# Graph-Machine-Learning-Group/sgp

Hardware: AMD Instinct MI355X
Metric: encoded node-steps/sec (higher is better)
Workload: dtype f32 (hop products: operands as fp16 hi + lo pairs, three 16-bit MFMA terms per product, fp32 accumulation -- agrees with fp32 to ~1e-7 of the operand scale; reservoir: recurrent products: state (|h| <= 1, x 2^14) and W_hh (per-row power-of-two scale) as two fp16 pieces (22 bits), hi*hi + hi*lo + lo*

## Files before the change

### include/sgp_amd.h

```cpp
#ifndef SGP_AMD_H
#define SGP_AMD_H

#include <stdint.h>

#ifdef __cplusplus
extern "C" {
#endif

#define SGP_ABI_VERSION 4

#define SGP_EINVAL   (-1)
#define SGP_EUNSUP   (-2)
#define SGP_ENOMEM   (-3)

#define SGP_ACT_TANH      0
#define SGP_ACT_RELU      1
#define SGP_ACT_SELF_NORM 2
#define SGP_ACT_IDENTITY  3
#define SGP_ACT_TANH_REL  4

typedef void* sgp_stream_t;

int sgp_abi_version(void);
const char* sgp_last_error(void);
const char* sgp_build_arch(void);

int64_t sgp_tune_value(const char* key, int64_t dflt);

int sgp_spmm_csr_f32(const int32_t* rowptr, const int32_t* col, const float* val,
                     const float* X, int64_t x_row_stride, int64_t x_batch_stride,
                     const float* X_halo, int64_t xh_row_stride, int64_t xh_batch_stride,
                     int32_t n_own,
                     float* Y, int64_t y_row_stride, int64_t y_batch_stride,
                     int32_t n_rows, int32_t n_cols, int32_t batch, int32_t feat,
                     const int32_t* pred, int32_t run_if, sgp_stream_t stream);

int sgp_spmm_tiled_f32(const int32_t* tile_row_ptr, const int32_t* uptr, const int32_t* ucol,
                       const int32_t* erow, const uint16_t* ecol, const float* eval,
                       int32_t tile_rows, int32_t n_tiles,
                       int32_t max_union, int32_t max_row_edges,
                       const float* X, int64_t x_row_stride, int64_t x_batch_stride,
                       const float* X_halo, int64_t xh_row_stride, int64_t xh_batch_stride,
                       int32_t n_own,
                       float* Y, int64_t y_row_stride, int64_t y_batch_stride,
                       int32_t n_rows, int32_t n_cols, int32_t batch, int32_t feat,
                       const int32_t* pred, int32_t run_if, sgp_stream_t stream);
int sgp_spmm_res_f32(const int32_t* uptr, const int32_t* ucol, const int32_t* usplit,
                     const int32_t* gptr, const int32_t* gsup, const int32_t* gidx, const float* gw,
                     const int32_t* rowmap,
                     int32_t n_tiles, int32_t max_union, int32_t max_tile_quads,
                     const float* X, int64_t x_row_stride, int64_t x_batch_stride,
                     const float* X_halo, int64_t xh_row_stride, int64_t xh_batch_stride,
                     int32_t n_own,
                     float* Y, int64_t y_row_stride, int64_t y_batch_stride,
                     int32_t n_rows, int32_t n_cols, int32_t batch, int32_t feat,
                     const int32_t* pred, int32_t run_if, sgp_stream_t stream);
int32_t sgp_spmm_res_max_union(void);
int32_t sgp_spmm_res_max_quads(void);
int sgp_spmm_res_tune(int32_t cfg);

int sgp_spmm_mix_f32(const int32_t* uptr, const int32_t* ucol, const int32_t* usplit,
                     const int32_t* gptr, const int32_t* gsup, const int32_t* gidx, const float* gw,
                     const int32_t* rowmap,
                     const int32_t* dptr, const int32_t* didx, const float* dw,
                     int32_t n_tiles, int32_t max_union, int32_t max_dense,
                     const float* X, int64_t x_row_stride, int64_t x_batch_stride,
                     const float* X_halo, int64_t xh_row_stride, int64_t xh_batch_stride,
                     int32_t n_own,
                     float* Y, int64_t y_row_stride, int64_t y_batch_stride,
                     int32_t n_rows, int32_t n_cols, int32_t batch, int32_t feat,
                     const int32_t* pred, int32_t run_if, sgp_stream_t stream);
int32_t sgp_spmm_mix_max_union(void);
int32_t sgp_spmm_mix_max_dense(int32_t halo);

int sgp_abs_max_f32(const float* X, int64_t x_row_stride, int64_t x_batch_stride,
                    int32_t n_rows, int32_t batch, int32_t feat, float* out, sgp_stream_t stream);


int sgp_col_stats_f32(const float* X, int64_t x_row_stride, int64_t x_batch_stride,
                      int32_t n_rows, int32_t batch, int32_t feat, int32_t t_stride, int32_t r_stride, int32_t accumulate,
                      float* stats, sgp_stream_t stream);

int sgp_split_prepare_f32(const float* stats, double n_samples, double s_eff, int32_t full,
                          const float* bound_in, float bound_scalar, float norm_inf, int32_t feat,
                          float* x_tab, float* bound_out, int32_t* flag, sgp_stream_t stream);

int sgp_spmm_split_f32(const int32_t* hdr, const int32_t* rowid, const int32_t* ucol, const void* afr,
                       const int32_t* adr, const float* rinv, int32_t n_tiles,
                       const float* X, int64_t x_row_stride, int64_t x_batch_stride,
                       const float* X_halo, int64_t xh_row_stride, int64_t xh_batch_stride, int32_t n_own,
                       float* Y, int64_t y_row_stride, int64_t y_batch_stride,
                       int32_t n_rows, int32_t n_cols, int32_t batch, int32_t feat,
                       const float* x_tab, int32_t accumulate, int32_t t_chunk, const int32_t* pred, int32_t run_if, sgp_stream_t stream);
int32_t sgp_spmm_split_chunks(void);
int32_t sgp_spmm_split_max_union(void);
int32_t sgp_spmm_split_waves(void);
int32_t sgp_spmm_split_rows_per_wave(void);
int32_t sgp_spmm_split_max_feat(void);

int sgp_spmm_split_banded_f32(const int32_t* hdr, const int32_t* rowid, const int32_t* ucol, const void* afr,
                              const int32_t* adr, const float* rinv, int32_t n_tiles,
                              const float* X, int64_t x_row_stride, int64_t x_batch_stride,
                              const float* X_halo, int64_t xh_row_stride, int64_t xh_batch_stride, int32_t n_own,
                              float* Y, int64_t y_row_stride, int64_t y_batch_stride,
                              int32_t n_rows, int32_t n_cols, int32_t batch, int32_t feat,
                              const float* x_tab, int32_t accumulate, int32_t t_chunk,
                              int32_t walk, const int32_t* band_first, int32_t n_bands,
                              const int32_t* pred, int32_t run_if, sgp_stream_t stream);

int sgp_spmm_split_wide_f32(const int32_t* hdr, const int32_t* rowid, const int32_t* ucol, const void* afr,
                            const int32_t* adr, const float* rinv, int32_t n_tiles,
                            const float* X, int64_t x_row_stride, int64_t x_batch_stride,
                            const float* X_halo, int64_t xh_row_stride, int64_t xh_batch_stride, int32_t n_own,
                            float* Y, int64_t y_row_stride, int64_t y_batch_stride,
                            int32_t n_rows, int32_t n_cols, int32_t batch, int32_t feat,
                            const float* x_tab, int32_t accumulate, int32_t t_chunk, const int32_t* pred, int32_t run_if, sgp_stream_t stream);
int sgp_spmm_split_wide_banded_f32(const int32_t* hdr, const int32_t* rowid, const int32_t* ucol, const void* afr,
                                   const int32_t* adr, const float* rinv, int32_t n_tiles,
                                   const float* X, int64_t x_row_stride, int64_t x_batch_stride,
                                   const float* X_halo, int64_t xh_row_stride, int64_t xh_batch_stride, int32_t n_own,
                                   float* Y, int64_t y_row_stride, int64_t y_batch_stride,
                                   int32_t n_rows, int32_t n_cols, int32_t batch, int32_t feat,
                                   const float* x_tab, int32_t accumulate, int32_t t_chunk,
                                   int32_t walk, const int32_t* band_first, int32_t n_bands,
                                   const int32_t* pred, int32_t run_if, sgp_stream_t stream);
int32_t sgp_spmm_split_wide_chunks(void);
int32_t sgp_spmm_split_wide_max_union(void);
int32_t sgp_spmm_split_wide_waves(void);
int32_t sgp_spmm_split_wide_rows_per_wave(void);
int32_t sgp_spmm_split_wide_max_feat(void);

int sgp_split_plan_order(const int64_t* rowptr, const int64_t* col, int64_t nnz, int64_t n_rows, int64_t n_cols,
                         int32_t waves, int32_t chunks, int32_t max_union, int32_t rows_per_wave, int64_t* order);
int64_t sgp_split_plan_deal(const int64_t* rowptr, const int64_t* col, int64_t nnz, int64_t n_rows, int64_t n_cols,
                            const int64_t* order, int64_t n_order,
                            int32_t waves, int32_t chunks, int32_t max_union, int32_t rows_per_wave,
                            int64_t* wave_of_row, int64_t* slot_of_row, int64_t* tile_of_wave, int64_t* rows_of_wave);
int sgp_split_plan_fill(const int64_t* rowptr, const int64_t* col, const float* val, int64_t nnz, int64_t n_rows, int64_t n_cols,
                        const int64_t* wave_of_row, const int64_t* slot_of_row, const int64_t* tile_of_wave,
                        const int64_t* rows_of_wave, int64_t n_waves, int64_t n_tiles,
                        int32_t waves, int32_t chunks, int32_t max_union,
                        int32_t* hdr, int32_t* rowid, int32_t* ucol, void* afr, int32_t* adr, float* rinv,
                        double* stats, int32_t threads);
int64_t sgp_split_plan_bands(const int32_t* ucol, int64_t n_tiles, int32_t max_union, int64_t n_cols,
                             int64_t col_budget, int32_t* band_first);

int sgp_spmm_colblock_f32(const int32_t* plan, const int32_t* segptr, const int32_t* wg_row0,
                          int32_t n_wg, int32_t n_blocks,
                          const float* X, int64_t x_row_stride, int64_t x_batch_stride,
                          const float* X_halo, int64_t xh_row_stride, int64_t xh_batch_stride, int32_t n_own,
                          float* Y, int64_t y_row_stride, int64_t y_batch_stride,
                          int32_t n_rows, int32_t n_cols, int32_t batch, int32_t feat,
                          const int32_t* pred, int32_t run_if, sgp_stream_t stream);
int32_t sgp_spmm_colblock_rows_cap(void);
int32_t sgp_spmm_colblock_round_pad(void);

int32_t sgp_spmm_tiled_max_union(int32_t feat);
int32_t sgp_spmm_tiled_max_tile_rows(void);
int32_t sgp_spmm_tiled_max_row_edges(void);

int sgp_spmm_tiled_form(int32_t tile_rows, int32_t max_row_edges, int32_t* rows_per_group, int32_t* batches);
int32_t sgp_spmm_csr_form(int32_t feat, int32_t aligned, int32_t predicated);

int64_t sgp_reservoir_workspace_bytes(int32_t F, int32_t R);
int sgp_reservoir_f32(const float* x, int64_t x_row_stride, int64_t x_step_stride,
                      const float* w_ih, const float* w_hh, const float* b,
                      double alpha, int32_t act,
                      float* out, int64_t out_row_stride, int64_t out_step_stride,
                      float* h_state, void* workspace,
                      int32_t T, int32_t N, int32_t F, int32_t R,
                      sgp_stream_t stream);

int sgp_reservoir_pieces_f32(const float* x, int64_t x_row_stride, int64_t x_step_stride,
                             const float* w_ih, const float* w_hh, const float* b,
                             double alpha, int32_t act,
                             float* out, int64_t out_row_stride, int64_t out_step_stride,
                             float* h_state, void* workspace,
                             int32_t t_piece, int32_t t_last, int32_t n_pieces,
                             int64_t x_piece_stride, int64_t out_piece_stride, int32_t no_store,
                             int32_t N, int32_t F, int32_t R,
                             const int32_t* pred, int32_t run_if, sgp_stream_t stream);

int sgp_reservoir_describe(int32_t F, int32_t R, int32_t N, int32_t T, int32_t act, double alpha, int32_t has_state,
                           int32_t n_pieces, int32_t no_store, int32_t has_pred,
                           int64_t x_row_stride, int64_t x_step_stride, int32_t x_align,
                           int64_t out_row_stride, int64_t out_step_stride, int32_t out_align,
                           char* text, int64_t capacity);

int64_t sgp_reservoir_fused_workspace_bytes(int32_t F, int32_t R, int32_t L);
int32_t sgp_reservoir_fused_supported(int32_t F, int32_t R, int32_t L);
int sgp_reservoir_fused_f32(const float* x, int64_t x_row_stride, int64_t x_step_stride,
                            const float* const* w_ih, const float* const* w_hh, const float* const* b,
                            const double* alpha, int32_t act,
                            float* out, int64_t out_row_stride, int64_t out_step_stride,
                            float* h_state, void* workspace,
                            int32_t T, int32_t N, int32_t F, int32_t R, int32_t L,
                            sgp_stream_t stream);
int sgp_reservoir_fused_sums_f32(const float* x, int64_t x_row_stride, int64_t x_step_stride,
                                 const float* const* w_ih, const float* const* w_hh, const float* const* b,
                                 const double* alpha, int32_t act,
                                 float* out, int64_t out_row_stride, int64_t out_step_stride,
                                 float* h_state, void* workspace, float* tile_sums,
                                 int32_t T, int32_t N, int32_t F, int32_t R, int32_t L,
                                 sgp_stream_t stream);

int32_t sgp_reservoir_window_supported(int32_t F, int32_t R, int32_t L);
int64_t sgp_reservoir_window_workspace_bytes(int32_t F, int32_t R, int32_t L, int32_t S, int64_t M);
int sgp_reservoir_window_f32(const float* x, int64_t x_batch_stride, int64_t x_step_stride, int64_t x_node_stride, int32_t Fx,
                             const float* u, int64_t u_batch_stride, int64_t u_step_stride, int64_t u_node_stride, int32_t Fu,
                             const int32_t* step_start,
                             const float* const* w_ih, const float* const* w_hh, const float* const* b,
                             const double* alpha, int32_t act,
                             const float* h0, float* out, int64_t out_row_stride,
                             void* workspace, int32_t packed,
                             int32_t B, int32_t N, int32_t S, int32_t R, int32_t L, sgp_stream_t stream);

int64_t sgp_gesn_workspace_bytes(int32_t N, int32_t R, int32_t L);
int sgp_gesn_tune(int32_t persistent);
int sgp_gesn_f32(const int32_t* rowptr, const int32_t* col, const float* val,
                 const float* x, int64_t x_row_stride, int64_t x_step_stride,
                 const float* const* w_ih, const float* const* w_hh, const float* const* b,
                 const double* alpha, int32_t act,
                 float* out, int64_t out_row_stride, int64_t out_step_stride,
                 float* h_state, void* workspace,
                 int32_t T, int32_t N, int32_t F, int32_t R, int32_t L, sgp_stream_t stream);
int sgp_gemm_nt_f32(const float* A, int64_t lda, const float* W, int64_t ldw, const float* bias,
                    float* C, int64_t ldc, int32_t M, int32_t N, int32_t K, sgp_stream_t stream);
int sgp_gesn_update_f32(const int32_t* rowptr, const int32_t* col, const float* val,
                        const float* z, const float* p, const float* h_in,
                        double alpha, int32_t act,
                        float* h_out, float* out_row, int64_t out_stride,
                        int32_t n_nodes, int32_t R, sgp_stream_t stream);

int sgp_node_mean_bcast_f32(const float* X, int64_t x_row_stride, int64_t x_batch_stride,
                            float* Y, int64_t y_row_stride, int64_t y_batch_stride,
                            float* partial,
                            int32_t n_rows, int32_t batch, int32_t feat,
                            sgp_stream_t stream);
int sgp_bcast_rows_f32(const float* src, float scale,
                       float* Y, int64_t y_row_stride, int64_t y_batch_stride,
                       int32_t n_rows, int32_t batch, int32_t feat,
                       sgp_stream_t stream);

int sgp_copy_rows_f32(const float* X, int64_t x_row_stride, int64_t x_batch_stride,
                      float* Y, int64_t y_row_stride, int64_t y_batch_stride,
                      int32_t n_rows, int32_t batch, int32_t feat,
                      sgp_stream_t stream);
int sgp_gather_rows_f32(const float* X, int64_t x_row_stride, int64_t x_batch_stride,
                        const int32_t* step, const int32_t* node, int32_t n_index,
                        float* out, int64_t out_row_stride, int64_t out_batch_stride,
                        int32_t batch, int32_t feat, sgp_stream_t stream);

int64_t sgp_grouped_linear_packed_floats(int32_t groups, int32_t ic, int32_t oc);
int sgp_grouped_linear_pack_f32(const float* w, float* packed, int32_t groups, int32_t ic, int32_t oc,
                                sgp_stream_t stream);
int sgp_grouped_linear_f32(const float* X, int64_t x_row_stride, int64_t x_batch_stride,
                           const int32_t* step, const int32_t* node,
                           const float* w_packed, const float* bias, int32_t act,
                           float* out, int64_t out_row_stride,
                           int32_t n_rows, int32_t groups, int32_t ic, int32_t oc,
                           sgp_stream_t stream);
int sgp_grouped_linear_fwd_f32(const float* X, int64_t x_row_stride, int64_t x_batch_stride,
                               const int32_t* step, const int32_t* node,
                               const float* w_packed, const float* bias, int32_t act,
                               float* out, int64_t out_row_stride, float* pre,
                               double dropout_p, uint64_t seed,
                               int32_t n_rows, int32_t groups, int32_t ic, int32_t oc,
                               sgp_stream_t stream);
int sgp_grouped_linear_dact_f32(const float* dy, int64_t dy_row_stride, const float* pre, int32_t act,
                                double dropout_p, uint64_t seed,
                                float* dz, int64_t n_rows, int32_t width, sgp_stream_t stream);
int sgp_grouped_linear_transpose_f32(const float* w, float* wt, int32_t groups, int32_t ic, int32_t oc,
                                     sgp_stream_t stream);
int sgp_grouped_linear_wgrad_f32(const float* X, int64_t x_row_stride, int64_t x_batch_stride,
                                 const int32_t* step, const int32_t* node,
                                 const float* dz, float* dw,
                                 int32_t n_rows, int32_t groups, int32_t ic, int32_t oc,
                                 sgp_stream_t stream);
int sgp_grouped_linear_form(int32_t ic, int32_t oc, int64_t x_row_stride, int64_t x_batch_stride, int32_t x_aligned16,
                            int32_t* jtc, int32_t* xvec);
int sgp_grouped_linear_wgrad_form(int32_t n_rows, int32_t groups, int32_t ic, int32_t oc,
                                  int32_t* rows_per_slice, int32_t* slices);

int64_t sgp_ridge_workspace_bytes(int32_t which, int64_t n_rows, int32_t n_cols, int32_t n_out);
int sgp_ridge_form(int32_t which, int64_t n_rows, int32_t n_cols, int32_t n_out, int64_t* out);

int sgp_ridge_colmeans_f32(const int64_t* segs, int32_t n_segs, const int32_t* steps, int64_t n_steps,
                           int64_t n_nodes, double* means, void* work, int64_t work_bytes, sgp_stream_t stream);

int sgp_ridge_gram_f32(const int64_t* segs, int32_t n_segs, const int32_t* steps, int64_t n_steps, int64_t n_nodes,
                       const float* shift, int32_t ones, double* gram, int64_t ldg, void* work, int64_t work_bytes,
                       sgp_stream_t stream);

int sgp_ridge_predict_score_f32(const int64_t* segs, int32_t n_segs, const int32_t* steps, int64_t n_steps,
                                int64_t n_nodes, const float* W, const double* b, int32_t horizon, int32_t channels,
                                const float* scale, const float* bias, int64_t sc_node_stride,
                                const float* y, int64_t y_ss, int64_t y_ns,
                                const uint8_t* mask, int64_t m_ss, int64_t m_ns, int64_t m_cs,
                                float* yhat, double* sums, void* work, int64_t work_bytes, sgp_stream_t stream);


int64_t sgp_dense_packed_floats(int32_t n_out, int32_t k);
int sgp_dense_pack_f32(const float* w, int64_t w_row_stride, int32_t transpose, int32_t n_out, int32_t k,
                       float* packed, sgp_stream_t stream);

int sgp_dense_f32(const float* X, int64_t x_row_stride, const int32_t* gather, int64_t row_mod,
                  const float* w_packed, const float* bias, int32_t n_rows, int32_t k, int32_t n_out,
                  int32_t act, int32_t n_act, int32_t dmode, const float* dpre, int64_t dpre_row_stride,
                  float* pre, int64_t pre_row_stride, double dropout_p, uint64_t seed, int64_t drop_width,
                  const float* add, int64_t add_row_stride,
                  float* out, const int64_t* out_map, sgp_stream_t stream);
int sgp_dense_form(int32_t n_rows, int32_t n_out, int32_t k, int64_t x_row_stride, int32_t x_aligned16,
                   int32_t* rows_per_wg, int32_t* xvec);

int64_t sgp_dense_wgrad_workspace_floats(int64_t n_rows, int32_t n_out, int32_t k, int32_t with_bias);
int sgp_dense_wgrad_f32(const float* dZ, int64_t dz_row_stride, const float* X, int64_t x_row_stride,
                        const int32_t* gather, int64_t row_mod, int32_t n_rows, int32_t n_out, int32_t k,
                        float* dw, int64_t dw_row_stride, float* db, float* work, int64_t work_floats,
                        sgp_stream_t stream);

int sgp_row_segsum_f32(const float* g, int64_t g_row_stride, int64_t n_rows, int32_t width,
                       const int32_t* perm, const int32_t* keys, int32_t n_seg, float* out, sgp_stream_t stream);


int sgp_multi_sqnorm_f32(const int64_t* table, int64_t n_chunks, const float* const* grads, double* partial,
                         float* norm_f32, double* norm_f64, sgp_stream_t stream);

int sgp_adam_step_f32(const int64_t* table, int64_t n_chunks, float* const* params, const float* const* grads,
                      float* const* exp_avg, float* const* exp_avg_sq, const float* norm, double max_norm,
                      double lr, double beta1, double beta2, double eps, double weight_decay, int64_t step,
                      int32_t decoupled, sgp_stream_t stream);

int64_t sgp_masked_metrics_workspace_doubles(int64_t batch, int32_t horizon, int64_t nodes, int32_t channels);
int sgp_masked_metrics_f32(const float* y_hat, const float* y, const uint8_t* mask, int64_t batch, int32_t horizon,
                           int64_t nodes, int32_t channels, const float* scale, const float* bias,
                           int64_t sc_node_stride, int32_t mask_nans, int32_t mask_inf, double* work,
                           int64_t work_doubles, double* state, sgp_stream_t stream);

int64_t sgp_masked_loss_workspace_doubles(int64_t batch, int32_t horizon, int64_t row, int32_t at);
int sgp_masked_loss_f32(const float* y_hat, const float* y, const uint8_t* mask, int64_t batch, int32_t horizon,
                        int64_t row, int32_t kind, int32_t at, int32_t mask_nans, double* work, int64_t work_doubles,
                        float* loss, double* count, sgp_stream_t stream);
int sgp_masked_loss_bwd_f32(const float* y_hat, const float* y, const uint8_t* mask, int64_t batch, int32_t horizon,
                            int64_t row, int32_t kind, int32_t at, int32_t mask_nans, const float* grad_out,
                            const double* count, float* grad, sgp_stream_t stream);


int32_t sgp_gated_gn_supported(int32_t H, int32_t act);
int32_t sgp_gated_gn_chunk_edges(void);
int64_t sgp_gated_gn_workspace_bytes(int32_t backward, int64_t b, int64_t n_edges, int64_t n_chunks, int32_t n_parts,
                                     int32_t H);

int sgp_gated_gn_edge_f32(const float* PQ, int64_t pq_row_stride, int32_t b, int32_t n, int32_t H, int32_t act,
                          const int32_t* chunks, int32_t n_chunks, const int32_t* src, int64_t n_edges,
                          const int32_t* fix, int32_t n_fix, int32_t n_parts,
                          const float* w2_packed, const float* b2, const float* wg, const float* bg,
                          float* agg, int64_t agg_row_stride, void* work, int64_t work_bytes, sgp_stream_t stream);

int sgp_gated_gn_edge_bwd_f32(const float* PQ, int64_t pq_row_stride, const float* dAgg, int64_t dagg_row_stride,
                              int32_t b, int32_t n, int32_t H, int32_t act,
                              const int32_t* chunks, int32_t n_chunks, const int32_t* src, int64_t n_edges,
                              const int32_t* fix, int32_t n_fix, int32_t n_parts,
                              const int32_t* src_ptr, const int32_t* src_pos,
                              const float* w2_packed, const float* w2t_packed, const float* b2, const float* wg,
                              const float* bg, float* dPQ, int64_t dpq_row_stride, float* dW2, float* db2, float* dwg,
                              float* dbg, void* work, int64_t work_bytes, sgp_stream_t stream);

int32_t sgp_rnn_window_supported(int32_t cell, int32_t H);
int64_t sgp_rnn_window_packed_floats(int32_t cell, int32_t H);
int64_t sgp_rnn_window_workspace_bytes(int32_t cell, int32_t H, int32_t S, int64_t M);
int sgp_rnn_window_pack_f32(const float* w_hh, int32_t cell, int32_t H, float* packed, sgp_stream_t stream);

int sgp_rnn_window_fwd_f32(int32_t cell, int32_t H, int32_t S, int64_t M, float* gates, const float* packed,
                           const float* b_hn, float* h_seq, float* c_seq, float* h_drop, double dropout_p, uint64_t seed,
                           float* h_last, int32_t save, sgp_stream_t stream);

int sgp_rnn_window_bwd_f32(int32_t cell, int32_t H, int32_t S, int64_t M, float* gates, const float* packed,
                           const float* h_seq, const float* c_seq, const float* dy, int32_t dy_full,
                           sgp_stream_t stream);

int32_t sgp_dcrnn_supported(int32_t H, int32_t k);

int sgp_diffuse_f32(const int32_t* rowptr0, const int32_t* col0, const float* val0, int64_t xcol0, int64_t ycol0,
                    const int32_t* rowptr1, const int32_t* col1, const float* val1, int64_t xcol1, int64_t ycol1,
                    const float* X, int64_t x_row_stride, int64_t x_batch_stride,
                    float* Y, int64_t y_row_stride, int64_t y_batch_stride,
                    int32_t n, int32_t batch, int32_t feat, int32_t accumulate, sgp_stream_t stream);

int sgp_dcrnn_gates_f32(const float* Dh, int64_t d_row_stride, const float* w_ru_packed,
                        const float* G, int64_t g_row_stride, float* ruc, int64_t ruc_row_stride,
                        float* Drh, int64_t drh_row_stride, int64_t R, int32_t H, int32_t k, sgp_stream_t stream);

int sgp_dcrnn_update_f32(const float* Drh, int64_t d_row_stride, const float* w_c_packed,
                         const float* G, int64_t g_row_stride, float* ruc, int64_t ruc_row_stride,
                         const float* h_prev, int64_t h_row_stride, float* h_seq_t, float* dh_next,
                         int64_t dh_next_row_stride, float* h_last, int64_t R, int32_t H, int32_t k,
                         sgp_stream_t stream);

int sgp_dcrnn_bwd_f32(int32_t phase, float* dh, const float* ruc, int64_t ruc_row_stride,
                      const float* h_prev, int64_t h_row_stride, const float* dDrh, int64_t ddrh_row_stride,
                      float* dz, int64_t dz_row_stride, int64_t R, int32_t H, sgp_stream_t stream);

int32_t sgp_gwnet_supported(int32_t H, int32_t Kt);

int sgp_gwnet_tconv_f32(const float* X, int64_t x_row_stride, int64_t x_rows, int64_t tap_rows,
                        const float* w_packed, const float* bias, float* Y, int64_t y_row_stride,
                        float* act, int64_t act_row_stride, int64_t n_rows, int32_t H, int32_t Kt,
                        sgp_stream_t stream);

int sgp_gwnet_tconv_bwd_f32(const float* dY, int64_t dy_row_stride, float* act, int64_t act_row_stride,
                            int64_t n_rows, int32_t H, sgp_stream_t stream);

int sgp_adj_apply_f32(const float* A, int64_t a_row_stride, int32_t transpose,
                      const float* X, int64_t xcol, int64_t x_row_stride, int64_t x_batch_stride,
                      float* Y, int64_t ycol, int64_t y_row_stride, int64_t y_batch_stride,
                      int32_t n, int32_t batch, int32_t feat, int32_t accumulate, sgp_stream_t stream);

int64_t sgp_adj_grad_workspace_floats(int32_t n, int32_t batch);
int sgp_adj_grad_f32(const float* dY, int64_t dycol, int64_t dy_row_stride, int64_t dy_batch_stride,
                     const float* X, int64_t xcol, int64_t x_row_stride, int64_t x_batch_stride,
                     float* dA, int64_t da_row_stride, int32_t n, int32_t batch, int32_t feat, int32_t accumulate,
                     float* work, int64_t work_floats, sgp_stream_t stream);

int sgp_row_softmax_f32(const float* L, int64_t l_row_stride, float* A, int64_t a_row_stride, int32_t n_rows, int32_t n,
                        sgp_stream_t stream);
int sgp_row_softmax_bwd_f32(const float* A, int64_t a_row_stride, const float* dA, int64_t da_row_stride,
                            const float* L, int64_t l_row_stride, float* dL, int64_t dl_row_stride,
                            int32_t n_rows, int32_t n, sgp_stream_t stream);

int64_t sgp_gwnet_norm_workspace_doubles(int64_t R, int32_t H);
int sgp_gwnet_norm_f32(int32_t kind, int32_t training, const float* Y, int64_t y_row_stride,
                       const float* res, int64_t res_row_stride, double dropout_p, uint64_t seed,
                       const float* weight, const float* bias, float* running_mean, float* running_var,
                       double momentum, double eps, float* z_save, float* stats,
                       float* out, int64_t out_row_stride, int64_t R, int32_t H,
                       double* work, int64_t work_doubles, sgp_stream_t stream);

int sgp_gwnet_norm_bwd_f32(int32_t kind, int32_t training, const float* dOut, int64_t dout_row_stride,
                           const float* z, const float* stats, const float* weight, double dropout_p, uint64_t seed,
                           double eps, float* dY, int64_t dy_row_stride, float* dRes, int64_t dres_row_stride,
                           float* dweight, float* dbias, int64_t R, int32_t H,
                           double* work, int64_t work_doubles, sgp_stream_t stream);

int sgp_subgraph_mark(const int32_t* ids, int64_t n_ids, uint64_t* mask, int64_t n_nodes, int32_t* err,
                      sgp_stream_t stream);
int sgp_subgraph_expand(const int32_t* src, const int32_t* dst, int64_t n_edges, const uint64_t* mask_in,
                        uint64_t* mask_out, int64_t n_nodes, sgp_stream_t stream);
int sgp_subgraph_edge_flags(const int32_t* src, const int32_t* dst, int64_t n_edges, const uint64_t* mask,
                            int64_t n_nodes, uint64_t* flags, uint8_t* edge_mask, sgp_stream_t stream);

int64_t sgp_compact_tiles(int64_t n);
int sgp_compact_pack_u8(const uint8_t* flags, int64_t n, uint64_t* bits, sgp_stream_t stream);
int sgp_compact_count(const uint64_t* bits, int64_t n, int32_t* tile_offsets, int32_t* total, sgp_stream_t stream);
int sgp_compact_scatter(const uint64_t* bits, int64_t n, const int32_t* tile_offsets, int64_t n_set, int32_t* idx32,
                        int64_t* idx64, int32_t* rank, sgp_stream_t stream);
int sgp_subgraph_edges(const uint64_t* flags, int64_t n_edges, const int32_t* tile_offsets, int64_t n_set,
                       const int32_t* src, const int32_t* dst, const float* weight, const int32_t* relabel,
                       int64_t n_nodes, int64_t* out_src, int64_t* out_dst, float* out_weight, sgp_stream_t stream);
int sgp_subgraph_take_edges(const int32_t* src, const int32_t* dst, const float* weight, int64_t n_edges,
                            const int32_t* pos, int64_t n_pos, const int64_t* keep, int64_t n_keep,
                            const int32_t* relabel, int64_t n_nodes, int64_t* out_src, int64_t* out_dst,
                            float* out_weight, int32_t* err, sgp_stream_t stream);

int32_t sgp_conn_max_knn(void);
int sgp_conn_geo_knn_f64(const double* unit, int64_t n, int32_t k, int32_t include_self, int32_t binary,
                         double threshold, double chord_zero, double scale, int32_t* out_col, double* out_val,
                         sgp_stream_t stream);
int sgp_conn_geo_rows_f64(const double* unit, int64_t n, int32_t include_self, int32_t binary, double threshold,
                          double chord_lo, double chord_hi, double scale, int32_t* row_count, const int64_t* rowptr,
                          int32_t* out_col, double* out_val, sgp_stream_t stream);
int sgp_conn_dense_knn(const void* sim, int32_t is_f64, int64_t row_stride, int64_t col_stride, int64_t n, int32_t k,
                       int32_t include_self, int32_t binary, double threshold, int32_t* out_col, double* out_val,
                       sgp_stream_t stream);
int sgp_conn_dense_rows(const void* sim, int32_t is_f64, int64_t row_stride, int64_t col_stride, int64_t n,
                        int32_t include_self, int32_t binary, double threshold, int32_t* row_count,
                        const int64_t* rowptr, int32_t* out_col, double* out_val, sgp_stream_t stream);
int sgp_correntropy_f32(const float* x, int64_t x_row_stride, int32_t n, int32_t period, int32_t n_chunks, double gamma,
                        float* norms, float* out, int64_t out_row_stride, sgp_stream_t stream);

int64_t sgp_scaler_workspace_bytes(int64_t m, int64_t g, int32_t regime, int64_t rows_per_wg);
int sgp_scaler_moments_f32(const float* x, const uint8_t* mask, int64_t mask_div, int64_t m, int64_t g, int32_t want_var,
                           int32_t regime, int64_t rows_per_wg, int32_t tile_cols, double* stats, void* ws,
                           int64_t ws_bytes, sgp_stream_t stream);
int sgp_scaler_select_f32(const float* x, const uint8_t* mask, int64_t mask_div, int64_t m, int64_t g, const double* stats,
                          double q_lo, double q_mid, double q_hi, int32_t regime, int64_t rows_per_wg, int32_t tile_cols,
                          float* ostat, void* ws, int64_t ws_bytes, sgp_stream_t stream);
int sgp_scaler_finish_f32(int32_t kind, const double* stats, const float* ostat, int64_t g, int32_t has_mask, double p0,
                          double p1, double adjust, float* bias, float* scale, sgp_stream_t stream);
int sgp_scaler_apply_f32(const float* x, float* out, const float* bias, const float* scale, int64_t n, int64_t n_params,
                         int32_t inverse, sgp_stream_t stream);

int32_t sgp_edge_sort_tile(void);
int32_t sgp_edge_sort_passes(int64_t n_nodes);
int64_t sgp_edge_sort_workspace_bytes(int64_t n_items);
int sgp_edge_sort(const void* keys, int32_t keys64, int64_t n_keys, const int32_t* payload_in, int64_t n_items,
                  int64_t n_nodes, int32_t* order, int32_t* ptr, int32_t* err, void* ws, int64_t ws_bytes,
                  sgp_stream_t stream);
int sgp_edge_segment_sum_f32(const int32_t* ptr, const int32_t* order, const float* weight, int64_t n_nodes,
                             int64_t n_items, float* deg, sgp_stream_t stream);
int sgp_edge_gather_f32(const int32_t* order, int64_t n_items, const void* other, int32_t other64, const float* weight,
                        const void* idx_a, const float* deg_a, const void* idx_b, const float* deg_b, int32_t idx64,
                        int64_t n_nodes, int32_t* col, float* val_a, float* val_b, sgp_stream_t stream);
int sgp_edge_chunk_tables(const int32_t* ptr, int64_t n_nodes, int32_t chunk, int32_t* scan, int32_t* counts,
                          int32_t* chunks, int64_t max_chunks, int32_t* fix, int64_t max_fix, sgp_stream_t stream);

#define SGP_SHIFT_GCN_NORM    1
#define SGP_SHIFT_SET_DIAG    2
#define SGP_SHIFT_REMOVE_DIAG 4
#define SGP_SHIFT_UNDIRECTED  8
#define SGP_SHIFT_TRANSPOSE   16
int64_t sgp_shift_operator_workspace_bytes(int64_t n_items, int64_t n_nodes);
int sgp_shift_operator_f32(const void* src, const void* dst, int32_t idx64, const float* weight, int64_t n_edges,
                           int64_t n_nodes, int32_t flags, int32_t* rowptr, int32_t* col, float* val, int64_t capacity,
                           int32_t* nnz, int32_t* err, void* ws, int64_t ws_bytes, sgp_stream_t stream);

#define SGP_SPGEMM_COUNT 1
#define SGP_SPGEMM_EMIT  2
#define SGP_SPGEMM_ERR_CAPACITY 1
#define SGP_SPGEMM_ERR_INDEX    2
int64_t sgp_spgemm_workspace_bytes(int64_t n_rows);
int sgp_spgemm_form(int64_t n_rows, int64_t n_cols, int64_t* out);
int sgp_spgemm_f32(const int32_t* a_rowptr, const int32_t* a_col, const float* a_val, int64_t a_capacity, int64_t n_rows,
                   int64_t n_mid, const int32_t* b_rowptr, const int32_t* b_col, const float* b_val, int64_t b_capacity,
                   int64_t n_cols, int32_t phase, int32_t* rowptr, int32_t* col, float* val, int64_t capacity,
                   int32_t* nnz, int32_t* err, void* ws, int64_t ws_bytes, sgp_stream_t stream);
int sgp_csr_take_rows_f32(const int32_t* a_rowptr, const int32_t* a_col, const float* a_val, int64_t a_capacity,
                          int64_t n_rows, const void* index, int32_t idx64, int64_t n_index, int32_t phase,
                          int32_t* rowptr, int32_t* col, float* val, int64_t capacity, int32_t* nnz, int32_t* err, void* ws,
                          int64_t ws_bytes, sgp_stream_t stream);

int sgp_event_create(void** ev);
int sgp_event_destroy(void* ev);
int sgp_event_record(void* ev, sgp_stream_t stream);
int sgp_event_elapsed_ms(void* start, void* stop, float* ms);

#ifdef __cplusplus
}
#endif
#endif
```

### sgp_amd/csrc/plan_split.hip

```cpp
#include "common.h"
#include <math.h>
#include <string.h>
#include <algorithm>
#include <atomic>
#include <new>
#include <system_error>
#include <thread>
#include <vector>

namespace {

constexpr int SET_SLOTS[4][8] = {{0, 1, 2, 3, 8, 9, 10, 11}, {4, 5, 6, 7, 12, 13, 14, 15},
                                 {16, 17, 18, 19, 24, 25, 26, 27}, {20, 21, 22, 23, 28, 29, 30, 31}};

inline uint16_t half_bits(_Float16 h) { uint16_t b; memcpy(&b, &h, 2); return b; }

inline void split_fp16(float v, uint16_t& hi, uint16_t& lo) {
    uint32_t bits;
    memcpy(&bits, &v, 4);
    bits &= 0xFFFFE000u;
    float hi32;
    memcpy(&hi32, &bits, 4);
    if (fabsf(v) < 6.103515625e-05f) hi32 = (float)(_Float16)v;
    const _Float16 h = (_Float16)hi32;
    const _Float16 l = (_Float16)(v - (float)h);
    hi = half_bits(h);
    lo = half_bits(l);
}

inline int row_exponent(float rmax) {
    if (!(rmax > 0.0f)) return 0;
    const float q = 16384.0f / rmax;
    int e;
    if (isinf(q)) e = 126;
    else { int ex; (void)frexpf(q, &ex); e = ex - 1; }
    return std::min(126, std::max(-126, e));
}

struct FillArgs {
    const int64_t* rowptr; const int64_t* col; const float* val;
    int64_t n_rows, n_cols;
    const int64_t* wave_of_row; const int64_t* slot_of_row; const int64_t* tile_of_wave; const int64_t* rows_of_wave;
    int64_t n_waves, n_tiles;
    int waves, chunks, max_union;
    int32_t* hdr; int32_t* rowid; int32_t* ucol; uint16_t* afr; int32_t* adr; float* rinv;
};

struct Scratch {
    std::vector<int32_t> stage_of_col, kpos_of_col;
    std::vector<int64_t> cols;
    std::vector<float> dense;
    explicit Scratch(const FillArgs& a) : stage_of_col(a.n_cols, -1), kpos_of_col(a.n_cols, -1), dense((size_t)a.chunks * 512) {}
};

int64_t fill_tile(const FillArgs& a, int64_t t, const int64_t* first_wave, const int64_t* row_list, const int64_t* row_first,
                  Scratch& s, int64_t& union_out) {
    const int W = a.waves, C = a.chunks;
    const int64_t w0 = first_wave[t], w1 = first_wave[t + 1];
    s.cols.clear();
    for (int64_t w = w0; w < w1; ++w)
        for (int64_t i = row_first[w]; i < row_first[w + 1]; ++i) {
            const int64_t r = row_list[i];
            s.cols.insert(s.cols.end(), a.col + a.rowptr[r], a.col + a.rowptr[r + 1]);
        }
    std::sort(s.cols.begin(), s.cols.end());
    s.cols.erase(std::unique(s.cols.begin(), s.cols.end()), s.cols.end());
    if (s.cols.empty()) s.cols.push_back(0);
    const int64_t U = (int64_t)s.cols.size();
    if (U > a.max_union) return -1;
    union_out = U;
    std::vector<int64_t> tile_cols(s.cols);
    for (int64_t i = 0; i < U; ++i) {
        s.stage_of_col[tile_cols[i]] = (int32_t)i;
        a.ucol[t * a.max_union + i] = (int32_t)tile_cols[i];
    }
    a.hdr[t * 64 + 2 * W] = (int32_t)U;
    int64_t keys = 0;
    for (int64_t w = w0; w < w1; ++w) {
        const int win = (int)(w - w0);
        const int nrows = (int)a.rows_of_wave[w];
        a.hdr[t * 64 + W + win] = nrows;
        s.cols.clear();
        for (int64_t i = row_first[w]; i < row_first[w + 1]; ++i) {
            const int64_t r = row_list[i];
            a.rowid[(t * W + win) * 16 + a.slot_of_row[r]] = (int32_t)r;
            s.cols.insert(s.cols.end(), a.col + a.rowptr[r], a.col + a.rowptr[r + 1]);
        }
        std::sort(s.cols.begin(), s.cols.end());
        s.cols.erase(std::unique(s.cols.begin(), s.cols.end()), s.cols.end());
        const int nk = (int)s.cols.size();
        if (nk > 32 * C) return -1;
        keys += nk;
        int32_t* adr = a.adr + ((t * W + win) * C) * 64;
        for (int c = 0; c < C; ++c) {
            int srow[32];
            for (int k = 0; k < 32; ++k) srow[k] = -1;
            const int k0 = 32 * c, k1 = std::min(nk, 32 * c + 32);
            int cnt_res[8] = {0, 0, 0, 0, 0, 0, 0, 0}, in_set[4] = {0, 0, 0, 0};
            int rank[32], slot[32];
            for (int k = k0; k < k1; ++k) rank[k - k0] = cnt_res[s.stage_of_col[s.cols[k]] & 7]++;
            for (int r = 0; r < 4; ++r)
                for (int res = 0; res < 8; ++res)
                    for (int k = k0; k < k1; ++k)
                        if (rank[k - k0] == r && (s.stage_of_col[s.cols[k]] & 7) == res) slot[k - k0] = SET_SLOTS[r][in_set[r]++];
            bool occ[32] = {};
            for (int k = k0; k < k1; ++k) if (rank[k - k0] < 4) occ[slot[k - k0]] = true;
            int free_at = 0;
            for (int res = 0; res < 8; ++res)
                for (int k = k0; k < k1; ++k)
                    if (rank[k - k0] >= 4 && (s.stage_of_col[s.cols[k]] & 7) == res) {
                        while (occ[free_at]) ++free_at;
                        slot[k - k0] = free_at;
                        occ[free_at] = true;
                    }
            for (int k = k0; k < k1; ++k) {
                srow[slot[k - k0]] = s.stage_of_col[s.cols[k]];
                s.kpos_of_col[s.cols[k]] = 32 * c + slot[k - k0];
            }
            for (int q = 0; q < 4; ++q) {
                int rep = -1;
                for (int i = 0; i < 8; ++i) { const int v = srow[SET_SLOTS[q][i]]; if (v >= 0 && (rep < 0 || v < rep)) rep = v; }
                if (rep < 0) rep = 0;
                for (int i = 0; i < 8; ++i) if (srow[SET_SLOTS[q][i]] < 0) srow[SET_SLOTS[q][i]] = rep;
            }
            for (int g = 0; g < 4; ++g)
                for (int li = 0; li < 16; ++li) {
                    unsigned av[2];
                    for (int j = 0; j < 2; ++j) {
                        const int sl = srow[8 * g + 4 * j + (li >> 2)];
                        av[j] = (unsigned)((sl >> 3) * 512 + (sl & 7) * 32 + 8 * (li & 3));
                    }
                    if (av[0] >= 65536u || av[1] >= 65536u) return -1;
                    adr[c * 64 + 16 * g + li] = (int32_t)(av[0] | (av[1] << 16));
                }
        }
        std::fill(s.dense.begin(), s.dense.end(), 0.0f);
        for (int64_t i = row_first[w]; i < row_first[w + 1]; ++i) {
            const int64_t r = row_list[i];
            const int sl = (int)a.slot_of_row[r];
            for (int64_t e = a.rowptr[r]; e < a.rowptr[r + 1]; ++e) {
                const int pos = s.kpos_of_col[a.col[e]];
                const int k = pos & 31;
                s.dense[(size_t)(pos >> 5) * 512 + (sl + 16 * (k >> 3)) * 8 + (k & 7)] += a.val[e];
            }
        }
        uint16_t* afr = a.afr + ((size_t)(t * W + win) * C) * 2 * 512;
        for (int sl = 0; sl < 16; ++sl) {
            float rmax = 0.0f;
            for (int c = 0; c < C; ++c)
                for (int g = 0; g < 4; ++g)
                    for (int e = 0; e < 8; ++e) rmax = std::max(rmax, fabsf(s.dense[(size_t)c * 512 + (sl + 16 * g) * 8 + e]));
            const int er = row_exponent(rmax);
            const float scale = ldexpf(1.0f, er);
            for (int c = 0; c < C; ++c)
                for (int g = 0; g < 4; ++g)
                    for (int e = 0; e < 8; ++e) {
                        const size_t at = (size_t)(sl + 16 * g) * 8 + e;
                        uint16_t hi, lo;
                        split_fp16(s.dense[(size_t)c * 512 + at] * scale, hi, lo);
                        afr[((size_t)c * 2 + 0) * 512 + at] = hi;
                        afr[((size_t)c * 2 + 1) * 512 + at] = lo;
                    }
            a.rinv[(t * W + win) * 16 + sl] = sl < nrows ? ldexpf(1.0f, -er) : 0.0f;
        }
    }
    return keys;
}

const char* rowptr_fault(const int64_t* rowptr, int64_t n_rows, int64_t nnz) {
    if (nnz < 0) return "negative nnz";
    if (n_rows > 0 && rowptr[0] != 0) return "rowptr[0] != 0";
    for (int64_t r = 0; r < n_rows; ++r)
        if (rowptr[r + 1] < rowptr[r]) return "rowptr decreases";
    if (n_rows > 0 && rowptr[n_rows] > nnz) return "rowptr[n_rows] > nnz";
    return nullptr;
}

template <class R, class F> R guarded(const char* what, F&& body) {
    try { return body(); }
    catch (const std::bad_alloc&) { return (R)sgp::fail(SGP_ENOMEM, "%s: out of host memory", what); }
    catch (const std::exception& e) { return (R)sgp::fail(SGP_EINVAL, "%s: %s", what, e.what()); }
    catch (...) { return (R)sgp::fail(SGP_EINVAL, "%s: unknown exception", what); }
}

}

extern "C" int64_t sgp_split_plan_deal(const int64_t* rowptr, const int64_t* col, int64_t nnz, int64_t n_rows, int64_t n_cols,
                                       const int64_t* order, int64_t n_order,
                                       int32_t waves, int32_t chunks, int32_t max_union, int32_t rows_per_wave,
                                       int64_t* wave_of_row, int64_t* slot_of_row, int64_t* tile_of_wave, int64_t* rows_of_wave) {
  return guarded<int64_t>("sgp_split_plan_deal", [&]() -> int64_t {
    if (!rowptr || (!col && nnz > 0) || !wave_of_row || !slot_of_row || !tile_of_wave || !rows_of_wave ||
        n_rows < 0 || n_cols < 0 || waves < 1 || chunks < 1 || max_union < 1 || rows_per_wave < 1 || (order && n_order < 0))
        return sgp::fail(SGP_EINVAL, "sgp_split_plan_deal: bad argument");
    if (const char* f = rowptr_fault(rowptr, n_rows, nnz)) return sgp::fail(SGP_EINVAL, "sgp_split_plan_deal: malformed CSR: %s", f);
    const int64_t cap = 32ll * chunks;
    std::vector<int64_t> wmark(n_cols, -1), tmark(n_cols, -1), c;
    for (int64_t r = 0; r < n_rows; ++r) wave_of_row[r] = slot_of_row[r] = -1;
    int64_t wave = -1, tile = -1, w_rows = 0, w_cols = 0, t_cols = 0, t_waves = 0;
    auto open_wave = [&](bool new_tile) {
        ++wave;
        if (new_tile) { ++tile; t_cols = t_waves = 0; }
        ++t_waves;
        w_rows = w_cols = 0;
        tile_of_wave[wave] = tile;
        rows_of_wave[wave] = 0;
    };
    const int64_t n_seq = order ? n_order : n_rows;
    for (int64_t i = 0; i < n_seq; ++i) {
        const int64_t r = order ? order[i] : i;
        if (r < 0 || r >= n_rows) return sgp::fail(SGP_EINVAL, "sgp_split_plan_deal: order entry out of range");
        if (wave_of_row[r] >= 0) return sgp::fail(SGP_EINVAL, "sgp_split_plan_deal: row %lld appears twice in the order", (long long)r);
        c.assign(col + rowptr[r], col + rowptr[r + 1]);
        std::sort(c.begin(), c.end());
        c.erase(std::unique(c.begin(), c.end()), c.end());
        const int64_t nc = (int64_t)c.size();
        if (nc > cap || nc > max_union) return -2;
        if (nc && (c.front() < 0 || c.back() >= n_cols)) return sgp::fail(SGP_EINVAL, "sgp_split_plan_deal: column out of range");
        if (wave < 0) open_wave(true);
        int64_t new_w = 0, new_t = 0;
        for (int64_t v : c) { new_w += wmark[v] != wave; new_t += tmark[v] != tile; }
        const bool need_wave = w_rows == rows_per_wave || w_cols + new_w > cap;
        if (t_cols + new_t > max_union || (need_wave && t_waves == waves)) { open_wave(true); new_w = new_t = nc; }
        else if (need_wave) { open_wave(false); new_w = nc; }
        for (int64_t v : c) { wmark[v] = wave; tmark[v] = tile; }
        w_cols += new_w;
        t_cols += new_t;
        wave_of_row[r] = wave;
        slot_of_row[r] = w_rows;
        rows_of_wave[wave] = ++w_rows;
    }
    return wave + 1;
  });
}

namespace {

struct OrderGraph {
    std::vector<int64_t> rp, cp;
    std::vector<int32_t> rc, cr;
    int32_t deg(int64_t r) const { return (int32_t)(rp[r + 1] - rp[r]); }
};

const char* order_graph(const int64_t* rowptr, const int64_t* col, int64_t n_rows, int64_t n_cols, OrderGraph& g) {
    g.rp.assign(n_rows + 1, 0);
    g.rc.reserve((size_t)rowptr[n_rows]);
    std::vector<int64_t> c;
    for (int64_t r = 0; r < n_rows; ++r) {
        c.assign(col + rowptr[r], col + rowptr[r + 1]);
        std::sort(c.begin(), c.end());
        c.erase(std::unique(c.begin(), c.end()), c.end());
        if (!c.empty() && (c.front() < 0 || c.back() >= n_cols)) return "column out of range";
        for (int64_t v : c) g.rc.push_back((int32_t)v);
        g.rp[r + 1] = (int64_t)g.rc.size();
    }
    g.cp.assign(n_cols + 1, 0);
    for (int32_t v : g.rc) ++g.cp[v + 1];
    for (int64_t v = 0; v < n_cols; ++v) g.cp[v + 1] += g.cp[v];
    g.cr.resize(g.rc.size());
    std::vector<int64_t> at(g.cp.begin(), g.cp.end() - 1);
    for (int64_t r = 0; r < n_rows; ++r)
        for (int64_t e = g.rp[r]; e < g.rp[r + 1]; ++e) g.cr[at[g.rc[e]]++] = (int32_t)r;
    return nullptr;
}

struct Orderer {
    const OrderGraph& g;
    const int64_t n_rows;
    const int32_t waves, wave_cols, max_union, rows_per_wave;
    std::vector<uint8_t> placed;
    std::vector<int32_t> t_mark, t_cnt, t_cnt_at, t_cand;
    std::vector<int32_t> w_mark, w_cnt, w_cnt_at, in_tile;
    std::vector<std::vector<int32_t>> bucket;
    std::vector<int32_t> rows, rest, wave_rows, wave_first;
    int32_t tile = -1, wave = -1, lo = 0;
    int64_t t_union = 0, w_union = 0, next_row = 0;

    Orderer(const OrderGraph& g_, int64_t n_rows_, int64_t n_cols, int32_t waves_, int32_t chunks, int32_t max_union_, int32_t rpw)
        : g(g_), n_rows(n_rows_), waves(waves_), wave_cols(32 * chunks), max_union(max_union_), rows_per_wave(rpw),
          placed(n_rows_, 0), t_mark(n_cols, -1), t_cnt(n_rows_, 0), t_cnt_at(n_rows_, -1), t_cand(n_rows_, -1),
          w_mark(n_cols, -1), w_cnt(n_rows_, 0), w_cnt_at(n_rows_, -1), in_tile(n_rows_, -1) {
        int32_t dmax = 0;
        for (int64_t r = 0; r < n_rows; ++r) dmax = std::max(dmax, g.deg(r));
        bucket.resize((size_t)dmax + 1);
    }
    int32_t t_have(int32_t r) const { return t_cnt_at[r] == tile ? t_cnt[r] : 0; }
    int32_t w_have(int32_t r) const { return w_cnt_at[r] == wave ? w_cnt[r] : 0; }
    void t_push(int32_t r) {
        const int32_t k = g.deg(r) - t_have(r);
        bucket[k].push_back(r);
        lo = std::min(lo, k);
    }
    void tile_take(int32_t r) {
        placed[r] = 1;
        rows.push_back(r);
        for (int64_t e = g.rp[r]; e < g.rp[r + 1]; ++e) {
            const int32_t c = g.rc[e];
            if (t_mark[c] == tile) continue;
            t_mark[c] = tile;
            ++t_union;
            for (int64_t i = g.cp[c]; i < g.cp[c + 1]; ++i) {
                const int32_t q = g.cr[i];
                if (placed[q]) continue;
                if (t_cnt_at[q] != tile) { t_cnt_at[q] = tile; t_cnt[q] = 0; }
                ++t_cnt[q];
                if (t_cand[q] == tile) t_push(q);
            }
            if (c < n_rows && !placed[c] && t_cand[c] != tile) { t_cand[c] = tile; t_push(c); }
        }
    }
    int32_t tile_best() {
        for (; lo < (int32_t)bucket.size(); ++lo) {
            std::vector<int32_t>& b = bucket[lo];
            size_t keep = 0;
            int32_t best = -1;
            for (int32_t q : b) {
                if (placed[q] || t_cand[q] != tile || g.deg(q) - t_have(q) != lo) continue;
                b[keep++] = q;
                if (best < 0 || t_have(q) > t_have(best) || (t_have(q) == t_have(best) && q < best)) best = q;
            }
            b.resize(keep);
            if (best >= 0) return best;
        }
        return -1;
    }
    void grow_tile() {
        ++tile;
        rows.clear();
        t_union = 0;
        for (auto& b : bucket) b.clear();
        lo = (int32_t)bucket.size();
        while (placed[next_row]) ++next_row;
        tile_take((int32_t)next_row);
        const size_t cap_rows = (size_t)waves * rows_per_wave;
        while (rows.size() < cap_rows) {
            int32_t r = tile_best();
            if (r < 0) {
                while (next_row < n_rows && placed[next_row]) ++next_row;
                if (next_row == n_rows) break;
                r = (int32_t)next_row;
            }
            if (t_union + g.deg(r) - t_have(r) > max_union) break;
            tile_take(r);
        }
    }
    void wave_take(int32_t r) {
        in_tile[r] = -1;
        wave_rows.push_back(r);
        for (int64_t e = g.rp[r]; e < g.rp[r + 1]; ++e) {
            const int32_t c = g.rc[e];
            if (w_mark[c] == wave) continue;
            w_mark[c] = wave;
            ++w_union;
            for (int64_t i = g.cp[c]; i < g.cp[c + 1]; ++i) {
                const int32_t q = g.cr[i];
                if (in_tile[q] != tile) continue;
                if (w_cnt_at[q] != wave) { w_cnt_at[q] = wave; w_cnt[q] = 0; }
                ++w_cnt[q];
            }
        }
    }
    int32_t cut_waves() {
        rest.assign(rows.begin(), rows.end());
        std::sort(rest.begin(), rest.end());
        for (int32_t r : rest) in_tile[r] = tile;
        wave_rows.clear();
        wave_first.assign(1, 0);
        while (!rest.empty()) {
            ++wave;
            w_union = 0;
            int32_t n_in = 0;
            size_t at = 0;
            for (;;) {
                const int32_t r = rest[at];
                rest.erase(rest.begin() + (int64_t)at);
                wave_take(r);
                if (++n_in == rows_per_wave || rest.empty()) break;
                at = 0;
                for (size_t i = 1; i < rest.size(); ++i) {
                    const int32_t q = rest[i], b = rest[at];
                    const int32_t nq = g.deg(q) - w_have(q), nb = g.deg(b) - w_have(b);
                    if (nq < nb || (nq == nb && w_have(q) > w_have(b))) at = i;
                }
                if (w_union + g.deg(rest[at]) - w_have(rest[at]) > wave_cols) break;
            }
            wave_first.push_back((int32_t)wave_rows.size());
        }
        return (int32_t)wave_first.size() - 1;
    }
    void run(int64_t* order) {
        int64_t n_out = 0;
        while (n_out < n_rows) {
            grow_tile();
            const int32_t n_waves = cut_waves();
            const int32_t kept = std::min(n_waves, waves);
            for (int32_t i = 0; i < wave_first[kept]; ++i) order[n_out++] = wave_rows[i];
            for (int32_t i = wave_first[kept]; i < wave_first[n_waves]; ++i) {
                placed[wave_rows[i]] = 0;
                next_row = std::min<int64_t>(next_row, wave_rows[i]);
            }
        }
    }
};

}

extern "C" int sgp_split_plan_order(const int64_t* rowptr, const int64_t* col, int64_t nnz, int64_t n_rows, int64_t n_cols,
                                    int32_t waves, int32_t chunks, int32_t max_union, int32_t rows_per_wave, int64_t* order) {
  return guarded<int>("sgp_split_plan_order", [&]() -> int {
    SGP_REQUIRE(rowptr && (col || nnz <= 0) && order, "sgp_split_plan_order: null pointer");
    SGP_REQUIRE(n_rows >= 0 && n_cols >= 0 && n_rows < (1ll << 31) - 1 && n_cols < (1ll << 31) - 1 && waves >= 1 && chunks >= 1 &&
                chunks <= (1 << 24) && max_union >= 1 && rows_per_wave >= 1 && (int64_t)waves * rows_per_wave < (1ll << 31),
                "sgp_split_plan_order: bad size");
    if (const char* f = rowptr_fault(rowptr, n_rows, nnz)) return sgp::fail(SGP_EINVAL, "sgp_split_plan_order: malformed CSR: %s", f);
    if (n_rows == 0) return 0;
    OrderGraph g;
    if (const char* f = order_graph(rowptr, col, n_rows, n_cols, g)) return sgp::fail(SGP_EINVAL, "sgp_split_plan_order: %s", f);
    Orderer(g, n_rows, n_cols, waves, chunks, max_union, rows_per_wave).run(order);
    return 0;
  });
}

extern "C" int sgp_split_plan_fill(const int64_t* rowptr, const int64_t* col, const float* val, int64_t nnz, int64_t n_rows, int64_t n_cols,
                                   const int64_t* wave_of_row, const int64_t* slot_of_row, const int64_t* tile_of_wave,
                                   const int64_t* rows_of_wave, int64_t n_waves, int64_t n_tiles,
                                   int32_t waves, int32_t chunks, int32_t max_union,
                                   int32_t* hdr, int32_t* rowid, int32_t* ucol, void* afr, int32_t* adr, float* rinv,
                                   double* stats, int32_t threads) {
  return guarded<int>("sgp_split_plan_fill", [&]() -> int {
    SGP_REQUIRE(rowptr && col && val && wave_of_row && slot_of_row && tile_of_wave && rows_of_wave && hdr && rowid && ucol &&
                afr && adr && rinv && stats, "sgp_split_plan_fill: null pointer");
    SGP_REQUIRE(n_rows > 0 && n_cols > 0 && n_waves > 0 && n_tiles > 0 && waves >= 1 && 2 * waves < 64 && chunks >= 1 &&
                max_union >= 1 && max_union <= 65536 / 64 * 8, "sgp_split_plan_fill: bad size");
    if (const char* f = rowptr_fault(rowptr, n_rows, nnz)) return sgp::fail(SGP_EINVAL, "sgp_split_plan_fill: malformed CSR: %s", f);
    for (int64_t e = 0; e < rowptr[n_rows]; ++e)
        SGP_REQUIRE(col[e] >= 0 && col[e] < n_cols, "sgp_split_plan_fill: column out of range");
    FillArgs a{rowptr, col, val, n_rows, n_cols, wave_of_row, slot_of_row, tile_of_wave, rows_of_wave, n_waves, n_tiles,
               waves, chunks, max_union, hdr, rowid, ucol, (uint16_t*)afr, adr, rinv};
    memset(hdr, 0, sizeof(int32_t) * 64 * n_tiles);
    std::fill(rowid, rowid + n_tiles * waves * 16, -1);
    std::fill(ucol, ucol + n_tiles * (int64_t)max_union, -1);
    memset(afr, 0, sizeof(uint16_t) * (size_t)n_tiles * waves * chunks * 2 * 512);
    memset(adr, 0, sizeof(int32_t) * (size_t)n_tiles * waves * chunks * 64);
    memset(rinv, 0, sizeof(float) * (size_t)n_tiles * waves * 16);
    std::vector<int64_t> first_wave(n_tiles + 1, 0), row_first(n_waves + 1, 0);
    for (int64_t w = 0; w < n_waves; ++w) {
        const int64_t t = tile_of_wave[w];
        SGP_REQUIRE(t >= 0 && t < n_tiles && (w == 0 || t == tile_of_wave[w - 1] || t == tile_of_wave[w - 1] + 1),
                    "sgp_split_plan_fill: tile_of_wave is not a non-decreasing run");
        SGP_REQUIRE(rows_of_wave[w] >= 0 && rows_of_wave[w] <= 16, "sgp_split_plan_fill: a wave holds at most 16 rows");
        ++first_wave[t + 1];
        row_first[w + 1] = row_first[w] + rows_of_wave[w];
    }
    for (int64_t t = 0; t < n_tiles; ++t) {
        SGP_REQUIRE(first_wave[t + 1] >= 1 && first_wave[t + 1] <= waves, "sgp_split_plan_fill: a tile holds 1 .. waves waves");
        first_wave[t + 1] += first_wave[t];
    }
    const int64_t n_dealt = row_first[n_waves];
    std::vector<int64_t> row_list(std::max<int64_t>(n_dealt, 1), -1);
    int64_t seen = 0;
    for (int64_t r = 0; r < n_rows; ++r) {
        const int64_t w = wave_of_row[r];
        if (w < 0) continue;
        SGP_REQUIRE(w < n_waves && slot_of_row[r] >= 0 && slot_of_row[r] < rows_of_wave[w] && row_list[row_first[w] + slot_of_row[r]] < 0,
                    "sgp_split_plan_fill: wave / slot of row %lld inconsistent", (long long)r);
        row_list[row_first[w] + slot_of_row[r]] = r;
        ++seen;
    }
    SGP_REQUIRE(seen == n_dealt, "sgp_split_plan_fill: rows_of_wave does not match wave_of_row");

    int nthr = threads > 0 ? threads : (int)std::thread::hardware_concurrency();
    nthr = (int)std::max<int64_t>(1, std::min<int64_t>(std::min(nthr, 64), n_tiles));
    nthr = (int)std::max<int64_t>(1, std::min<int64_t>(nthr, (1ll << 30) / (8 * n_cols)));
    std::atomic<int64_t> next(0), keys(0), usum(0), umax(0);
    std::atomic<int> bad(0);
    auto work = [&]() {
        try {
            Scratch s(a);
            int64_t k_local = 0, u_local = 0, u_max = 0;
            for (;;) {
                const int64_t t = next.fetch_add(1);
                if (t >= n_tiles || bad.load()) break;
                int64_t U = 0;
                const int64_t k = fill_tile(a, t, first_wave.data(), row_list.data(), row_first.data(), s, U);
                if (k < 0) { bad.store(1); break; }
                k_local += k; u_local += U; u_max = std::max(u_max, U);
            }
            keys += k_local; usum += u_local;
            int64_t cur = umax.load();
            while (u_max > cur && !umax.compare_exchange_weak(cur, u_max)) {}
        } catch (...) { bad.store(2); }
    };
    if (nthr == 1) work();
    else {
        std::vector<std::thread> pool;
        pool.reserve(nthr);
        try {
            for (int i = 0; i < nthr; ++i) pool.emplace_back(work);
        } catch (const std::system_error&) {
            if (pool.empty()) work();
        }
        for (auto& th : pool) th.join();
    }
    if (bad.load() == 2) return sgp::fail(SGP_ENOMEM, "sgp_split_plan_fill: out of host memory");
    if (bad.load()) return sgp::fail(SGP_EUNSUP, "sgp_split_plan_fill: the dealt rows break the kernel's limits");
    double norm_inf = 0.0;
    for (int64_t r = 0; r < n_rows; ++r) {
        double sum = 0.0;
        for (int64_t e = rowptr[r]; e < rowptr[r + 1]; ++e) sum += fabs((double)val[e]);
        norm_inf = std::max(norm_inf, sum);
    }
    const double dealt = (double)std::max<int64_t>(1, n_dealt);
    stats[0] = (double)n_tiles; stats[1] = (double)n_waves; stats[2] = (double)n_dealt / (double)n_waves;
    stats[3] = dealt / (double)n_tiles; stats[4] = (double)usum.load() / dealt;
    stats[5] = (double)keys.load() / ((double)n_waves * chunks * 32); stats[6] = (double)umax.load(); stats[7] = norm_inf;
    return 0;
  });
}

extern "C" int64_t sgp_split_plan_bands(const int32_t* ucol, int64_t n_tiles, int32_t max_union, int64_t n_cols,
                                        int64_t col_budget, int32_t* band_first) {
  return guarded<int64_t>("sgp_split_plan_bands", [&]() -> int64_t {
    if (!ucol || !band_first || n_tiles < 1 || n_tiles >= (1ll << 31) || max_union < 1 || n_cols < 1 || col_budget < 1)
        return sgp::fail(SGP_EINVAL, "sgp_split_plan_bands: bad argument");
    std::vector<int64_t> mark(n_cols, -1);
    int64_t band = 0, b_cols = 0;
    band_first[0] = 0;
    for (int64_t t = 0; t < n_tiles; ++t) {
        const int32_t* u = ucol + t * max_union;
        int64_t fresh = 0, U = 0;
        for (; U < max_union && u[U] >= 0; ++U) {
            if (u[U] >= n_cols) return sgp::fail(SGP_EINVAL, "sgp_split_plan_bands: column out of range");
            fresh += mark[u[U]] != band;
        }
        if (t > band_first[band] && b_cols + fresh > col_budget) {
            band_first[++band] = (int32_t)t;
            b_cols = 0;
            fresh = U;
        }
        for (int64_t i = 0; i < U; ++i) mark[u[i]] = band;
        b_cols += fresh;
    }
    band_first[band + 1] = (int32_t)n_tiles;
    return band + 1;
  });
}
```

### sgp_amd/csrc/spmm_split_impl.h

```cpp
#include "common.h"
#include <stdlib.h>
#include <type_traits>

namespace {

typedef _Float16 h8 __attribute__((ext_vector_type(8)));
typedef short s4v __attribute__((ext_vector_type(4)));
using sgp::f32x4;

#ifndef SGP_SPLIT_NW
#define SGP_SPLIT_NW 16
#endif
constexpr int NW = SGP_SPLIT_NW;
static_assert(NW == 8 || NW == 12 || NW == 16, "8, 12 or 16 waves x 16 rows");
#ifndef SGP_SPLIT_NCH
#define SGP_SPLIT_NCH 7
#endif
constexpr int NCH = SGP_SPLIT_NCH;
#ifndef SGP_SPLIT_SMAX
#define SGP_SPLIT_SMAX 768
#endif
constexpr int SMAX = SGP_SPLIT_SMAX;
constexpr int NLD = (SMAX + 16 * NW - 1) / (16 * NW);
constexpr int BUF = SMAX * 64;
#ifndef SGP_SPLIT_VSTAGE
#define SGP_SPLIT_VSTAGE 0
#endif
constexpr bool VSTAGE = SGP_SPLIT_VSTAGE != 0;
constexpr int NBUF = VSTAGE ? 2 : 3;
constexpr int HDR = 64;
constexpr int MAXFEAT = 1024;
#ifndef SGP_SPLIT_CR
#define SGP_SPLIT_CR 3
#endif
constexpr int CR = SGP_SPLIT_CR;
static_assert(BUF < 65536 - 512, "packed 16-bit transpose-read addresses");
static_assert(VSTAGE ? (CR >= 1 && CR + NLD <= NCH) : (CR >= NLD - 1 && CR + NLD < NCH),
              "conversion sits between the staging requests and the last chunk");
static_assert(NLD <= 7 && NBUF * BUF + 2 * MAXFEAT * 4 <= 160 * 1024, "three buffers and the scale table in 160 KB");

#ifndef SGP_SPLIT_RING
#define SGP_SPLIT_RING 3
#endif
constexpr int RING = SGP_SPLIT_RING;
static_assert(RING >= 2 && RING <= 4, "one to three chunks of operands in flight");

constexpr int conv_ops(int c) {
    if (VSTAGE) return (c == CR - 1 ? 1 : 0) + (c >= CR && c < CR + NLD ? 2 : 0);
    return c == CR ? 2 : (c > CR && c < CR + NLD ? 3 : (c == CR + NLD ? 2 : 0));
}
#ifndef SGP_SPLIT_ACC3
#define SGP_SPLIT_ACC3 0
#endif
#ifndef SGP_SPLIT_SPREAD
#define SGP_SPLIT_SPREAD 0
#endif
constexpr bool SPREAD = SGP_SPLIT_SPREAD != 0;
constexpr int lgkm_behind(int c, bool conv) {
    int n = 4 * ((c + RING - 1 < NCH ? c + RING - 1 : NCH - 1) - c);
    if (SPREAD && c + RING - 1 < NCH) n -= 2;
    if (conv) for (int j = (c - (RING - 1) > 0 ? c - (RING - 1) : 0); j < c; ++j) n += conv_ops(j);
    return n;
}
constexpr int lgkm_wait(int c, bool conv) { return lgkm_behind(c, conv) < 15 ? lgkm_behind(c, conv) : 15; }
static_assert(RING == 4 || (lgkm_behind(NCH - 1, true) <= 15 && lgkm_behind(CR + 1, true) <= 15 && lgkm_behind(CR + 2, true) <= 15),
              "the standard ring's waits are exact");

template <int I, int N, class F> __device__ __forceinline__ void static_for(F&& f) {
    if constexpr (I < N) { f(std::integral_constant<int, I>{}); static_for<I + 1, N>(f); }
}

#ifdef SGP_ABLATION
#define ABL(bit) ((a.mode & (bit)) != 0)
#else
#define ABL(bit) false
#endif

struct SplitArgs {
    const int* hdr; const int* rowid; const int* ucol; const h8* afr; const int* adr; const float* rinv;
    int n_tiles, tiles_per_xcd;
    int time_major;
    const int* bands; int n_bands;
    int chunks_per_xcd;
    const float* X; long long xrs, xbs;
    const float* XH; long long xhrs, xhbs;
    int n_own;
    float* Y; long long yrs, ybs;
    int batch, nslice, t_chunk;
    const float* xtab;
    const int* pred; int pred_want;
    unsigned long long* dbg;
    int mode;
};

struct BOp { s4v h0, h1, l0, l1; };
__device__ __forceinline__ void tr_issue(BOp& b, unsigned a0, unsigned a1) {
    asm volatile("ds_read_b64_tr_b16 %0, %4\n\tds_read_b64_tr_b16 %1, %5\n\t"
                 "ds_read_b64_tr_b16 %2, %4 offset:256\n\tds_read_b64_tr_b16 %3, %5 offset:256"
                 : "=&v"(b.h0), "=&v"(b.h1), "=&v"(b.l0), "=&v"(b.l1) : "v"(a0), "v"(a1) : "memory");
}
__device__ __forceinline__ void tr_issue_hi(BOp& b, unsigned a0, unsigned a1) {
    asm volatile("ds_read_b64_tr_b16 %0, %2\n\tds_read_b64_tr_b16 %1, %3" : "=&v"(b.h0), "=&v"(b.h1) : "v"(a0), "v"(a1) : "memory");
}
__device__ __forceinline__ void tr_issue_lo(BOp& b, unsigned a0, unsigned a1) {
    asm volatile("ds_read_b64_tr_b16 %0, %2 offset:256\n\tds_read_b64_tr_b16 %1, %3 offset:256" : "=&v"(b.l0), "=&v"(b.l1) : "v"(a0), "v"(a1) : "memory");
}
template <int N> __device__ __forceinline__ void tr_wait(BOp& b) {
    asm volatile("s_waitcnt lgkmcnt(%4)" : "+v"(b.h0), "+v"(b.h1), "+v"(b.l0), "+v"(b.l1) : "n"(N));
}
__device__ __forceinline__ h8 cat8(s4v x, s4v y) {
    return __builtin_bit_cast(h8, __builtin_shufflevector(x, y, 0, 1, 2, 3, 4, 5, 6, 7));
}
__device__ __forceinline__ unsigned addr_lo(unsigned base, unsigned packed) {
    unsigned r;
    asm("v_add_u32_sdwa %0, %1, %2 dst_sel:DWORD dst_unused:UNUSED_PAD src0_sel:DWORD src1_sel:WORD_0" : "=v"(r) : "v"(base), "v"(packed));
    return r;
}
__device__ __forceinline__ unsigned addr_hi(unsigned base, unsigned packed) {
    unsigned r;
    asm("v_add_u32_sdwa %0, %1, %2 dst_sel:DWORD dst_unused:UNUSED_PAD src0_sel:DWORD src1_sel:WORD_1" : "=v"(r) : "v"(base), "v"(packed));
    return r;
}

__device__ __forceinline__ void lds_read16(f32x4& v, unsigned addr) {
    asm volatile("ds_read_b128 %0, %1" : "=&v"(v) : "v"(addr) : "memory");
}
template <int OFF> __device__ __forceinline__ void lds_read16_off(f32x4& v, unsigned addr) {
    asm volatile("ds_read_b128 %0, %1 offset:%2" : "=&v"(v) : "v"(addr), "n"(OFF) : "memory");
}
template <int OFF> __device__ __forceinline__ void lds_write8(unsigned addr, uint2 d) {
    asm volatile("ds_write_b64 %0, %1 offset:%2" :: "v"(addr), "v"(d), "n"(OFF) : "memory");
}

__device__ __forceinline__ void dma16(unsigned voff, const void* sbase, unsigned lds_off) {
    asm volatile("s_mov_b32 m0, %2\n\ts_nop 0\n\tglobal_load_lds_dwordx4 %0, %1"
                 :: "v"(voff), "s"(sbase), "s"(lds_off) : "memory");
}
__device__ __forceinline__ void dma16_vaddr(const void* vaddr, unsigned lds_off) {
    asm volatile("s_mov_b32 m0, %1\n\ts_nop 0\n\tglobal_load_lds_dwordx4 %0, off" :: "v"(vaddr), "s"(lds_off) : "memory");
}

__device__ __forceinline__ void vload16(f32x4& d, unsigned voff, const void* sbase) {
    asm volatile("global_load_dwordx4 %0, %1, %2" : "=&v"(d) : "v"(voff), "s"(sbase) : "memory");
}
__device__ __forceinline__ void vload16_vaddr(f32x4& d, const void* vaddr) {
    asm volatile("global_load_dwordx4 %0, %1, off" : "=&v"(d) : "v"(vaddr) : "memory");
}

#ifndef SGP_SPLIT_STORE_MOD
#define SGP_SPLIT_STORE_MOD ""
#endif
template <int OFF> __device__ __forceinline__ void store16(const void* sbase, unsigned voff, f32x4 d) {
    asm volatile("global_store_dwordx4 %0, %1, %2 offset:%3 " SGP_SPLIT_STORE_MOD :: "v"(voff), "v"(d), "s"(sbase), "n"(OFF) : "memory");
}

template <int N> __device__ __forceinline__ void wait_vm() { asm volatile("s_waitcnt vmcnt(%0)" :: "n"(N) : "memory"); }
__device__ __forceinline__ void wait_vm_n(int n) {
    switch (n) {
        case 0: wait_vm<0>(); break; case 1: wait_vm<1>(); break; case 2: wait_vm<2>(); break;
        case 3: wait_vm<3>(); break; case 4: wait_vm<4>(); break; case 5: wait_vm<5>(); break;
        case 6: wait_vm<6>(); break; default: wait_vm<7>(); break;
    }
}

__device__ __forceinline__ void split4(const f32x4 v, const f32x4 s, uint2& hi, uint2& lo) {
    unsigned h01, h23, l01, l23;
    asm("v_fma_mixlo_f16 %0, %1, %2, 0" : "=v"(h01) : "v"(v[0]), "v"(s[0]));
    asm("v_fma_mixhi_f16 %0, %1, %2, 0" : "+v"(h01) : "v"(v[1]), "v"(s[1]));
    asm("v_fma_mixlo_f16 %0, %1, %2, 0" : "=v"(h23) : "v"(v[2]), "v"(s[2]));
    asm("v_fma_mixhi_f16 %0, %1, %2, 0" : "+v"(h23) : "v"(v[3]), "v"(s[3]));
    asm("v_fma_mixlo_f16 %0, %1, %2, -%3 op_sel_hi:[0,0,1]" : "=&v"(l01) : "v"(v[0]), "v"(s[0]), "v"(h01));
    asm("v_fma_mixhi_f16 %0, %1, %2, -%3 op_sel:[0,0,1] op_sel_hi:[0,0,1]" : "+v"(l01) : "v"(v[1]), "v"(s[1]), "v"(h01));
    asm("v_fma_mixlo_f16 %0, %1, %2, -%3 op_sel_hi:[0,0,1]" : "=&v"(l23) : "v"(v[2]), "v"(s[2]), "v"(h23));
    asm("v_fma_mixhi_f16 %0, %1, %2, -%3 op_sel:[0,0,1] op_sel_hi:[0,0,1]" : "+v"(l23) : "v"(v[3]), "v"(s[3]), "v"(h23));
    hi.x = h01; hi.y = h23; lo.x = l01; lo.y = l23;
}

template <bool HALO, bool ACC>
__global__ __launch_bounds__(NW * 64, NW / 4) void spmm_split(SplitArgs a) {
    extern __shared__ __attribute__((aligned(16))) char lds[];
    if (a.pred != nullptr && a.pred[0] != a.pred_want) return;

    const int xcd = blockIdx.x & 7, j = blockIdx.x >> 3;
    int tile = a.time_major ? j % a.n_tiles : xcd * a.tiles_per_xcd + j % a.tiles_per_xcd;
    int tchunk = a.time_major ? (j / a.n_tiles) * 8 + xcd : j / a.tiles_per_xcd;
    if (a.time_major == 2) {
        int lo = 0, hi = a.n_bands;
        while (hi - lo > 1) {
            const int mid = (lo + hi) >> 1;
            if (a.bands[mid] * a.chunks_per_xcd <= j) lo = mid; else hi = mid;
        }
        const int t0 = a.bands[lo], nt = a.bands[lo + 1] - t0, jj = j - t0 * a.chunks_per_xcd;
        if (nt <= 0 || jj < 0) return;
        tile = t0 + jj % nt;
        tchunk = (jj / nt) * 8 + xcd;
    }
    if (tile < 0 || tile >= a.n_tiles) return;
    const int t_begin = tchunk * a.t_chunk;
    const int t_end = min(a.batch, t_begin + a.t_chunk);
    if (t_begin >= t_end) return;

    const int tid = threadIdx.x, lane = tid & 63;
    const int wave = __builtin_amdgcn_readfirstlane(tid >> 6);
    const int src_tile = ABL(16) ? xcd * a.tiles_per_xcd : tile;
    const int nU = __builtin_amdgcn_readfirstlane(a.hdr[(size_t)src_tile * HDR + 2 * NW]);
    const unsigned lds0 = (unsigned)(size_t)(__attribute__((address_space(3))) char*)lds;
    const int feat = a.nslice * 16;

    {
        float* tab = (float*)(lds + NBUF * BUF);
        for (int i = tid; i < 2 * feat; i += NW * 64) tab[i] = a.xtab[i];
    }
    h8 af[NCH][2];
    unsigned ad[NCH];
    {
        const h8* ap = a.afr + ((size_t)(tile * NW + wave) * NCH * 2) * 64 + lane;
        const int* dp = a.adr + ((size_t)(tile * NW + wave) * NCH) * 64 + lane;
#pragma unroll
        for (int c = 0; c < NCH; ++c) {
            af[c][0] = ap[(c * 2 + 0) * 64];
            af[c][1] = ap[(c * 2 + 1) * 64];
            ad[c] = (unsigned)dp[c * 64];
        }
    }
    unsigned xoff[NLD];
    const int* uc = a.ucol + (size_t)src_tile * SMAX;
    int nld = 0;
#pragma unroll
    for (int i = 0; i < NLD; ++i) {
        const int s = (i * NW + wave) * 16 + (lane >> 2);
        const int c = uc[s < nU ? s : 0];
        if (HALO && c >= a.n_own)
            xoff[i] = 0x80000000u | ((unsigned)(c - a.n_own) * (unsigned)a.xhrs * 4u + (unsigned)(lane & 3) * 16u);
        else
            xoff[i] = (unsigned)c * (unsigned)a.xrs * 4u + (unsigned)(lane & 3) * 16u;
        if ((i * NW + wave) * 16 < nU) nld = i + 1;
    }
    const int* rid = a.rowid + (size_t)(tile * NW + wave) * 16;
    const int row_a = rid[lane & 15];
    const float rinv = a.rinv[(size_t)(tile * NW + wave) * 16 + (lane & 15)];
    const unsigned yo = row_a < 0 ? ~0u : (unsigned)row_a * (unsigned)a.yrs * 4u + 16u * (unsigned)(lane >> 4);
    __builtin_amdgcn_s_waitcnt(0x0F70);
    const unsigned own = lds0 + wave * 1024 + lane * 16;
    const unsigned cv_off = lds0 + wave * 1024 + (lane >> 5) * 512 + ((lane >> 2) & 7) * 32 + (lane & 3) * 8;
    const unsigned tab_cv = lds0 + NBUF * BUF + (lane & 3) * 16;
    const unsigned tab_rs = lds0 + NBUF * BUF + feat * 4 + (lane >> 4) * 16;

    auto piece = [&](unsigned off, const float* xb, const float* xh, unsigned lds_off) {
        if constexpr (HALO) {
            const char* b = (off & 0x80000000u) ? (const char*)xh : (const char*)xb;
            dma16_vaddr(b + (off & 0x7fffffffu), lds_off);
        } else {
            dma16(off, xb, lds_off);
        }
    };
    auto issue_dma = [&](int t, int sl, int buf) {
        const float* xb = ABL(64) ? a.X : a.X + (long long)t * a.xbs + sl * 16;
        const float* xh = HALO ? a.XH + (long long)t * a.xhbs + sl * 16 : nullptr;
        const unsigned base = lds0 + buf * BUF + wave * 1024;
#pragma unroll
        for (int i = 0; i < NLD; ++i)
            if (i < nld) piece(xoff[i], xb, xh, base + i * (NW * 1024));
    };

    const int n_units = (t_end - t_begin) * a.nslice;
    int dt = t_begin, dsl = 0;
    auto advance = [&](int& t, int& sl) { if (++sl == a.nslice) { sl = 0; ++t; } };

    f32x4 ld[VSTAGE ? NLD : 1];
#pragma unroll
    for (int i = 0; i < (VSTAGE ? NLD : 1); ++i) ld[i] = f32x4{0, 0, 0, 0};
    auto vpiece = [&](f32x4& d, unsigned off, const float* xb, const float* xh) {
        if constexpr (HALO) {
            const char* b = (off & 0x80000000u) ? (const char*)xh : (const char*)xb;
            vload16_vaddr(d, b + (off & 0x7fffffffu));
        } else {
            vload16(d, off, xb);
        }
    };
    auto issue_loads = [&](int t, int sl) {
        const float* xb = a.X + (long long)t * a.xbs + sl * 16;
        const float* xh = HALO ? a.XH + (long long)t * a.xhbs + sl * 16 : nullptr;
        static_for<0, (VSTAGE ? NLD : 0)>([&](auto I) {
            constexpr int i = decltype(I)::value;
            vpiece(ld[i], xoff[i], xb, xh);
        });
    };
    if constexpr (VSTAGE) {
        asm volatile("s_waitcnt lgkmcnt(0)\n\ts_barrier" ::: "memory");
        issue_loads(dt, dsl); advance(dt, dsl);
        f32x4 s4;
        lds_read16(s4, tab_cv);
        wait_vm<0>();
        static_for<0, NLD>([&](auto I) {
            constexpr int i = decltype(I)::value;
            asm volatile("s_waitcnt lgkmcnt(0)" : "+v"(s4), "+v"(ld[i]) :: "memory");
            uint2 hi, lo;
            split4(ld[i], s4, hi, lo);
            lds_write8<i * NW * 1024>(cv_off, hi); lds_write8<i * NW * 1024 + 256>(cv_off, lo);
        });
        if (n_units <= 1) { dt = t_begin; dsl = 0; }
        issue_loads(dt, dsl); advance(dt, dsl);
        if (n_units <= 2) { dt = t_begin; dsl = 0; }
        asm volatile("s_waitcnt lgkmcnt(0)\n\ts_barrier" ::: "memory");
    } else {
        issue_dma(dt, dsl, 0); advance(dt, dsl);
        if (n_units > 1) { issue_dma(dt, dsl, 1); advance(dt, dsl); wait_vm_n(nld); } else wait_vm<0>();
        asm volatile("s_waitcnt lgkmcnt(0)\n\ts_barrier" ::: "memory");
        {
            f32x4 v[NLD], s4;
            lds_read16(s4, tab_cv);
#pragma unroll
            for (int i = 0; i < NLD; ++i) lds_read16(v[i], own + i * (NW * 1024));
            asm volatile("s_waitcnt lgkmcnt(0)" : "+v"(s4), "+v"(v[0]), "+v"(v[NLD - 1]), "+v"(v[NLD / 2]));
            static_for<0, NLD>([&](auto I) {
                constexpr int i = decltype(I)::value;
                uint2 hi, lo;
                split4(v[i], s4, hi, lo);
                lds_write8<i * NW * 1024>(cv_off, hi); lds_write8<i * NW * 1024 + 256>(cv_off, lo);
            });
        }
        asm volatile("s_waitcnt lgkmcnt(0)\n\ts_barrier" ::: "memory");

    }

    int t = t_begin, sl = 0;
    unsigned cur = 0, nxt = BUF, nn = 2 * BUF;
    f32x4 h0 = {0, 0, 0, 0};
    auto stamp = [&](int u, int k) {
        if (ABL(256) && blockIdx.x == 0 && lane == 0 && u >= 16 && u < 24)
            a.dbg[((u - 16) * NW + wave) * 8 + k] = __builtin_amdgcn_s_memtime();
    };
    const float* xb2 = ABL(64) ? a.X : a.X + (long long)dt * a.xbs + dsl * 16;
    const float* xh2 = HALO ? a.XH + (long long)dt * a.xhbs + dsl * 16 : nullptr;
    const long long x_wrap = a.xbs - 16 * (a.nslice - 1), xh_wrap = a.xhbs - 16 * (a.nslice - 1);
    float* ys = a.Y + (long long)t * a.ybs;
    const long long y_wrap = a.ybs - 16 * (a.nslice - 1);
    int sl1 = a.nslice > 1 ? 1 : 0;
    for (int u = 0; u < n_units; ++u) {
        stamp(u, 0);
        const bool dma_now = u + 2 < n_units && !ABL(1);
        const unsigned base2 = lds0 + nn + wave * 1024;
        const unsigned cbo = lds0 + cur;

        f32x4 acc0 = {0, 0, 0, 0}, acc1 = {0, 0, 0, 0};
#if SGP_SPLIT_ACC3
        f32x4 acc2 = {0, 0, 0, 0};
#endif
        f32x4 v, s4;
        BOp b[RING];
        stamp(u, 1);
#pragma unroll
        for (int c = 0; c < RING - 1; ++c) tr_issue(b[c], addr_lo(cbo, ad[c]), addr_hi(cbo, ad[c]));
        static_for<0, NCH>([&](auto C) {
            constexpr int c = decltype(C)::value;
            BOp& x = b[c % RING];
            unsigned na0 = 0, na1 = 0;
            if constexpr (c + RING - 1 < NCH) {
                na0 = addr_lo(cbo, ad[c + RING - 1]); na1 = addr_hi(cbo, ad[c + RING - 1]);
                if constexpr (SPREAD) tr_issue_hi(b[(c + RING - 1) % RING], na0, na1);
                else tr_issue(b[(c + RING - 1) % RING], na0, na1);
            }
            if (ABL(8)) tr_wait<lgkm_wait(c, false)>(x); else tr_wait<lgkm_wait(c, true)>(x);
            if (!ABL(2)) {
                const h8 bh = cat8(x.h0, x.h1), bl = cat8(x.l0, x.l1);
                acc0 = __builtin_amdgcn_mfma_f32_16x16x32_f16(bh, af[c][0], acc0, 0, 0, 0);
                if constexpr (SPREAD && c + RING - 1 < NCH) tr_issue_lo(b[(c + RING - 1) % RING], na0, na1);
                acc1 = __builtin_amdgcn_mfma_f32_16x16x32_f16(bl, af[c][0], acc1, 0, 0, 0);
#if SGP_SPLIT_ACC3
                acc2 = __builtin_amdgcn_mfma_f32_16x16x32_f16(bh, af[c][1], acc2, 0, 0, 0);
#else
                acc1 = __builtin_amdgcn_mfma_f32_16x16x32_f16(bh, af[c][1], acc1, 0, 0, 0);
#endif
            } else if constexpr (SPREAD && c + RING - 1 < NCH) tr_issue_lo(b[(c + RING - 1) % RING], na0, na1);
            if constexpr (VSTAGE) {
                if constexpr (c == CR - 1) lds_read16(s4, tab_cv + sl1 * 64);
                if constexpr (c >= CR && c < CR + NLD) {
                    constexpr int i = c - CR;
                    wait_vm<NLD - 1>();
                    if constexpr (i == 0) asm volatile("s_waitcnt lgkmcnt(%2)" : "+v"(s4), "+v"(ld[i]) : "n"(c + RING - 1 < NCH ? 4 : 0) : "memory");
                    else asm volatile("" : "+v"(ld[i]) :: "memory");
                    uint2 hi, lo;
                    split4(ld[i], s4, hi, lo);
                    const unsigned w = cv_off + nxt;
                    lds_write8<i * NW * 1024>(w, hi); lds_write8<i * NW * 1024 + 256>(w, lo);
                    vpiece(ld[i], xoff[i], xb2, xh2);
                }
            } else {
            if constexpr (c < NLD) { if (dma_now && c < nld) piece(xoff[c], xb2, xh2, base2 + c * (NW * 1024)); }
            }
            if constexpr (!VSTAGE && c >= CR && c <= CR + NLD) {
                if (!ABL(8)) {
                    constexpr int i = c - CR;
                    if constexpr (i == 0) {
                        if (dma_now) wait_vm_n(nld); else wait_vm<0>();
                        lds_read16(s4, tab_cv + sl1 * 64);
                    } else {
                        asm volatile("s_waitcnt lgkmcnt(%2)" : "+v"(s4), "+v"(v) : "n"(c + RING - 1 < NCH ? 4 : 0));
                        uint2 hi, lo;
                        split4(v, s4, hi, lo);
                        const unsigned w = cv_off + nxt;
                        lds_write8<(i - 1) * NW * 1024>(w, hi); lds_write8<(i - 1) * NW * 1024 + 256>(w, lo);
                    }
                    if constexpr (i < NLD) lds_read16_off<i * NW * 1024>(v, own + nxt);
                }
            }
        });
        stamp(u, 3);
        if (!ABL(4)) {
            f32x4 iv;
            lds_read16(iv, tab_rs + sl * 64);
            asm volatile("s_waitcnt lgkmcnt(0)" : "+v"(iv));
#if SGP_SPLIT_ACC3
            acc1 += acc2;
#endif
            const f32x4 r0 = (acc0 + acc1) * (iv * rinv);
            if (!(sl & 1) && sl + 1 < a.nslice && !ABL(32)) {
                h0 = r0;
            } else if (yo != ~0u) {
                if constexpr (ACC) {
                    char* yb = (char*)ys + yo;
                    if ((sl & 1) && !ABL(32)) { *(f32x4*)(yb - 64) += h0; *(f32x4*)yb += r0; }
                    else *(f32x4*)yb += r0;
                } else {
                    if ((sl & 1) && !ABL(32)) { store16<-64>(ys, yo, h0); store16<0>(ys, yo, r0); }
                    else store16<0>(ys, yo, r0);
                }
            }
        }
        stamp(u, 5);
        if (VSTAGE ? u + 3 < n_units : dma_now) {
            const bool wrap = ++dsl == a.nslice;
            if (wrap) dsl = 0;
            if (!ABL(64)) xb2 += wrap ? x_wrap : 16;
            if (HALO) xh2 += wrap ? xh_wrap : 16;
        }
        {
            const bool wrap = sl + 1 == a.nslice;
            ys += wrap ? y_wrap : 16;
            sl = sl1;
            sl1 = sl1 + 1 == a.nslice ? 0 : sl1 + 1;
            if (wrap) ++t;
        }
        if constexpr (VSTAGE) { const unsigned f = cur; cur = nxt; nxt = f; }
        else { const unsigned f = cur; cur = nxt; nxt = nn; nn = f; }
        asm volatile("s_waitcnt lgkmcnt(0)\n\ts_barrier" ::: "memory");
        stamp(u, 6);
    }
}

}

extern "C" int32_t SGP_SPLIT_NAME(chunks)(void) { return NCH; }
extern "C" int32_t SGP_SPLIT_NAME(max_union)(void) { return SMAX; }
extern "C" int32_t SGP_SPLIT_NAME(waves)(void) { return NW; }
extern "C" int32_t SGP_SPLIT_NAME(rows_per_wave)(void) { return 16; }
extern "C" int32_t SGP_SPLIT_NAME(max_feat)(void) { return MAXFEAT; }

namespace {
int launch_split(const char* entry, const int32_t* hdr, const int32_t* rowid, const int32_t* ucol, const void* afr,
                 const int32_t* adr, const float* rinv, int32_t n_tiles, const sgp::HopOperands& o,
                 const float* x_tab, int32_t accumulate, int32_t t_chunk,
                 int32_t walk, const int32_t* band_first, int32_t n_bands) {
    const int32_t n_rows = o.n_rows, n_cols = o.n_cols, batch = o.batch, feat = o.feat;
    SGP_REQUIRE(n_tiles >= 0 && batch >= 0 && n_rows >= 0 && n_cols >= 0, "%s: negative size", entry);
    if (n_tiles == 0 || batch == 0 || n_rows == 0) return 0;
    SGP_REQUIRE(walk >= 0 && walk <= 3, "%s: walk = %d (0 chosen here, 1 tile-major, 2 time-major, 3 banded)", entry, walk);
    SGP_REQUIRE(walk != 3 || (band_first != nullptr && n_bands >= 1 && n_bands <= n_tiles),
                "%s: band table of %d bands for %d tiles", entry, n_bands, n_tiles);
    SGP_REQUIRE(hdr && rowid && ucol && afr && adr && rinv && x_tab, "%s: null pointer", entry);
    if (int rc = sgp::check_hop_operands(entry, o, {1ll << 29, 1ll << 29, 1ll << 30, true, 16, SGP_EINVAL, false})) return rc;
    SGP_REQUIRE(feat > 0 && feat <= MAXFEAT, "%s: feat = %d outside 16 .. %d (the scale table's LDS)", entry, feat, MAXFEAT);
    SplitArgs a;
    a.hdr = hdr; a.rowid = rowid; a.ucol = ucol; a.afr = (const h8*)afr; a.adr = adr; a.rinv = rinv;
    a.n_tiles = n_tiles; a.tiles_per_xcd = (n_tiles + 7) / 8;
    a.X = o.X; a.xrs = o.xrs; a.xbs = o.xbs;
    a.XH = o.Xh; a.xhrs = o.xhrs; a.xhbs = o.xhbs; a.n_own = o.Xh ? o.n_own : 0x7fffffff;
    a.Y = o.Y; a.yrs = o.yrs; a.ybs = o.ybs;
    a.batch = batch; a.nslice = feat / 16;
    a.xtab = x_tab; a.pred = o.pred; a.pred_want = o.run_if;
    const bool auto_tc = t_chunk <= 0;
    if (t_chunk <= 0) {
        int cus = 256, dev = 0;
        if (hipGetDevice(&dev) != hipSuccess || hipDeviceGetAttribute(&cus, hipDeviceAttributeMultiprocessorCount, dev) != hipSuccess || cus < 1)
            cus = 256;
        double best = 1e30;
        for (int tc = 64; tc >= 8; tc >>= 1) {
            if (tc > batch && tc > 8) continue;
            const double w = (double)n_tiles * ((batch + tc - 1) / tc) / cus;
            const double cost = (w <= 1.0 ? 1.0 / w : (double)(long long)(w + 0.999999) / w) * (1.0 + 1.6 / tc);
            if (cost < best - 1e-9) { best = cost; t_chunk = tc; }
        }
        if (t_chunk <= 0) t_chunk = 8;
    }
    static const long tm_tune = sgp::tune("split_time_major", -1);
    static const long tm_tc = sgp::tune("split_tc", 0);
    a.time_major = tm_tune >= 0 ? (int)(tm_tune != 0) : (int)((long long)n_cols * feat * 4 <= (4ll << 20) && n_tiles >= 8);
    a.bands = nullptr; a.n_bands = 0; a.chunks_per_xcd = 0;
    if (walk != 0) a.time_major = walk - 1;
    if (walk == 3) { a.bands = band_first; a.n_bands = n_bands; }
    if (a.time_major) {
        if (tm_tc > 0 && auto_tc) t_chunk = (int)tm_tc;
        else if (auto_tc && a.time_major == 1 && n_tiles <= 32 && t_chunk > 16) t_chunk = 16;
        else if (auto_tc && a.time_major == 2 && t_chunk > 32) t_chunk = 32;
    }
    a.t_chunk = t_chunk;
#ifdef SGP_ABLATION
    static const int abl = (int)sgp::tune("split_abl", 0);
#else
    constexpr int abl = 0;
#endif
    a.mode = abl;
    a.dbg = nullptr;
    if (abl & 256) { if (hipMalloc(&a.dbg, 8 * NW * 8 * 8) != hipSuccess) return sgp::fail(SGP_EINVAL, "dbg alloc"); (void)hipMemset(a.dbg, 0, 8 * NW * 8 * 8); }
    const int n_tchunks = (batch + t_chunk - 1) / t_chunk;
    a.chunks_per_xcd = (n_tchunks + 7) / 8;
    SGP_REQUIRE(8ll * n_tiles * a.chunks_per_xcd < (1ll << 31), "spmm_split: %d tiles x %d time chunks beyond one launch", n_tiles, n_tchunks);
    auto kern = o.Xh ? (accumulate ? spmm_split<true, true> : spmm_split<true, false>)
                       : (accumulate ? spmm_split<false, true> : spmm_split<false, false>);
    const int lds_bytes = NBUF * BUF + 2 * feat * 4;
    hipError_t e = hipFuncSetAttribute((const void*)kern, hipFuncAttributeMaxDynamicSharedMemorySize, NBUF * BUF + 2 * MAXFEAT * 4);
    if (e != hipSuccess) return sgp::fail((int)e, "spmm_split: LDS attribute: %s", hipGetErrorString(e));
    const unsigned grid = a.time_major ? 8u * (unsigned)n_tiles * (unsigned)((n_tchunks + 7) / 8)
                                       : 8u * (unsigned)a.tiles_per_xcd * (unsigned)n_tchunks;
    hipLaunchKernelGGL(kern, dim3(grid), dim3(NW * 64), lds_bytes, (hipStream_t)o.stream, a);
    if (abl & 256) {
        unsigned long long h[8 * NW * 8];
        (void)hipDeviceSynchronize();
        (void)hipMemcpy(h, a.dbg, sizeof(h), hipMemcpyDeviceToHost);
        (void)hipFree(a.dbg);
        printf("spmm_split timeline (cycles since the unit's top; columns: top | chunk loop start | - | chunk loop done | - | stores | barrier)\n");
        for (int u = 0; u < 8; ++u) for (int w = 0; w < NW; ++w) {
            const unsigned long long* r = h + (u * NW + w) * 8;
            printf("  unit %d wave %d: top %llu |", u, w, r[0] - h[0]);
            for (int k = 1; k < 7; ++k) printf(" %6lld", (long long)(r[k] - r[0]));
            printf("\n");
        }
    }
    return sgp::check_launch("spmm_split");
}
}

extern "C" int SGP_SPLIT_NAME(f32)(const int32_t* hdr, const int32_t* rowid, const int32_t* ucol, const void* afr,
                                  const int32_t* adr, const float* rinv,
                                  int32_t n_tiles,
                                  const float* X, int64_t x_row_stride, int64_t x_batch_stride,
                                  const float* X_halo, int64_t xh_row_stride, int64_t xh_batch_stride, int32_t n_own,
                                  float* Y, int64_t y_row_stride, int64_t y_batch_stride,
                                  int32_t n_rows, int32_t n_cols, int32_t batch, int32_t feat,
                                  const float* x_tab, int32_t accumulate, int32_t t_chunk, const int32_t* pred, int32_t run_if, sgp_stream_t stream) {
    return launch_split(SGP_STR(SGP_SPLIT_NAME(f32)), hdr, rowid, ucol, afr, adr, rinv, n_tiles,
                        {X, x_row_stride, x_batch_stride, X_halo, xh_row_stride, xh_batch_stride, n_own, Y, y_row_stride,
                         y_batch_stride, n_rows, n_cols, batch, feat, pred, run_if, stream},
                        x_tab, accumulate, t_chunk, 0, nullptr, 0);
}

extern "C" int SGP_SPLIT_NAME(banded_f32)(const int32_t* hdr, const int32_t* rowid, const int32_t* ucol, const void* afr,
                                         const int32_t* adr, const float* rinv,
                                         int32_t n_tiles,
                                         const float* X, int64_t x_row_stride, int64_t x_batch_stride,
                                         const float* X_halo, int64_t xh_row_stride, int64_t xh_batch_stride, int32_t n_own,
                                         float* Y, int64_t y_row_stride, int64_t y_batch_stride,
                                         int32_t n_rows, int32_t n_cols, int32_t batch, int32_t feat,
                                         const float* x_tab, int32_t accumulate, int32_t t_chunk,
                                         int32_t walk, const int32_t* band_first, int32_t n_bands,
                                         const int32_t* pred, int32_t run_if, sgp_stream_t stream) {
    return launch_split(SGP_STR(SGP_SPLIT_NAME(banded_f32)), hdr, rowid, ucol, afr, adr, rinv, n_tiles,
                        {X, x_row_stride, x_batch_stride, X_halo, xh_row_stride, xh_batch_stride, n_own, Y, y_row_stride,
                         y_batch_stride, n_rows, n_cols, batch, feat, pred, run_if, stream},
                        x_tab, accumulate, t_chunk, walk, band_first, n_bands);
}
```

### sgp_amd/csrc/spmm_split_wide.hip

```cpp
#define SGP_SPLIT_NW 8
#define SGP_SPLIT_NCH 14
#define SGP_SPLIT_SMAX 896
#define SGP_SPLIT_CR 6
#define SGP_SPLIT_VSTAGE 1
#define SGP_SPLIT_NAME(x) sgp_spmm_split_wide_##x
#include "spmm_split_impl.h"
```

### sgp_amd/graph.py

```python
from typing import NamedTuple

import numpy as np
import torch

from . import hip, tune
from .tileplan import build_reordered_plan, build_tile_plan, locality_order


def _as_edge_tensors(edge_index, edge_weight):
    if isinstance(edge_index, np.ndarray):
        edge_index = torch.from_numpy(edge_index)
        if edge_weight is not None and isinstance(edge_weight, np.ndarray):
            edge_weight = torch.from_numpy(edge_weight)
    if not torch.is_tensor(edge_index):
        raise RuntimeError("Edge index must be (edge_index, edge_weight) tuple "
                           "or SparseTensor.")
    ei = edge_index.detach().to("cpu", torch.long)
    ew = None if edge_weight is None else edge_weight.detach().to("cpu", torch.float32)
    return ei, ew


def _coalesce(row, col, val, n):
    key = row * n + col
    uniq, inv = torch.unique(key, sorted=True, return_inverse=True)
    out = torch.zeros(uniq.numel(), dtype=val.dtype).index_add_(0, inv, val)
    return uniq // n, uniq % n, out


class _Operands(NamedTuple):
    batch: int
    fits32: bool
    split_layout: bool
    halo_aligned: bool
    bound: str


_NOMINAL = _Operands(batch=4, fits32=True, split_layout=True, halo_aligned=True, bound="measured")


def _split_layout_ok(t):
    return t.is_cuda and t.stride(1) % 4 == 0 and t.stride(0) % 4 == 0 and t.data_ptr() % 16 == 0 and \
        t.shape[1] * max(t.stride(1), 1) < 2 ** 29


def _rows32(t):
    return t.shape[1] * max(t.stride(1), 1) < 2 ** 30


def _operands(x, y, halo, x_bound):
    number = isinstance(x_bound, (int, float))
    bound = "measured" if x_bound is None or (number and x_bound == 0) else \
        "nonfinite" if number and not (0 < x_bound < float("inf")) else "finite"
    return _Operands(x.shape[0],
                     _rows32(x) and _rows32(y) and (halo is None or _rows32(halo)),
                     _split_layout_ok(x) and _split_layout_ok(y) and (halo is None or _split_layout_ok(halo)),
                     halo is None or (halo.stride(1) % 4 == 0 and halo.stride(0) % 4 == 0 and halo.data_ptr() % 16 == 0),
                     bound)


class _Choice(NamedTuple):
    kernel: str = None
    plan: object = None
    split: object = None
    lazy: bool = False
    tile: object = None
    error: Exception = None
    walk: object = None


SPLIT_TIME_MAJOR_BYTES = 4 << 20
SPLIT_BAND_BYTES = 4 << 20
SPLIT_BANDED_DEFAULT = "on"


def split_band_cols(n_cols, feat, n_tiles):
    mode = tune.get("split_banded", SPLIT_BANDED_DEFAULT)
    if mode == "off" or feat <= 0:
        return None
    if mode == "on":
        if n_cols * feat * 4 <= SPLIT_TIME_MAJOR_BYTES and n_tiles >= 8:
            return None
        budget = SPLIT_BAND_BYTES
    else:
        try:
            budget = int(mode)
        except ValueError:
            raise ValueError(f"SGP_TUNE: split_banded={mode!r} is not off, on or a byte count") from None
        if budget <= 0:
            return None
    return max(1, budget // (feat * 4))


_LAUNCH = {
    "spmm_mix": hip.spmm_mix,
    "spmm_res": hip.spmm_res,
    "spmm_colblock": hip.spmm_colblock,
    "spmm_tiled": hip.spmm_tiled,
    "spmm_csr_rows": lambda csr, *args, **kw: hip.spmm_csr(*csr, *args, **kw),
}


class ShiftOperator:

    def __init__(self, rowptr, col, val, num_nodes, num_cols=None):
        self.rowptr = rowptr.to(torch.int32).contiguous()
        self.col = col.to(torch.int32).contiguous()
        self.val = val.to(torch.float32).contiguous()
        self.num_nodes = int(num_nodes)
        self.num_cols = int(num_nodes if num_cols is None else num_cols)
        self._dev = {}
        self._plans = {}
        self._exact_seen = False
        self._flag_host, self._flag_pending = None, []

    @classmethod
    def from_coo(cls, row, col, val, num_nodes, gcn_norm=False, set_diag=False,
                 remove_diag=False):
        n = int(num_nodes)
        row, col, val = _coalesce(row, col, val, n)
        if set_diag or remove_diag:
            keep = row != col
            row, col, val = row[keep], col[keep], val[keep]
        if set_diag:
            idx = torch.arange(n, dtype=torch.long)
            row, col = torch.cat([row, idx]), torch.cat([col, idx])
            val = torch.cat([val, torch.ones(n, dtype=val.dtype)])
            order = torch.argsort(row * n + col)
            row, col, val = row[order], col[order], val[order]
        deg = torch.zeros(n, dtype=torch.float32).index_add_(0, row, val)
        if gcn_norm:
            d = deg.pow(-0.5)
            d[d == float("inf")] = 0
            val = d[row] * val * d[col]
        else:
            d = deg.pow(-1.0)
            d[d == float("inf")] = 0
            val = d[row] * val
        counts = torch.bincount(row, minlength=n)
        rowptr = torch.zeros(n + 1, dtype=torch.long)
        rowptr[1:] = torch.cumsum(counts, 0)
        return cls(rowptr, col, val, n)

    @classmethod
    def from_edges(cls, edge_index, edge_weight=None, num_nodes=None, gcn_norm=False,
                   set_diag=False, remove_diag=False, undirected=False, transpose=False):
        ei, ew = _as_edge_tensors(edge_index, edge_weight)
        n = int(num_nodes) if num_nodes is not None else (int(ei.max()) + 1 if ei.numel() else 0)
        if ei.numel() and (int(ei.min()) < 0 or int(ei.max()) >= n):
            raise ValueError("edge_index out of range for num_nodes")
        if ew is None:
            ew = torch.ones(ei.shape[1], dtype=torch.float32)
        col, row = ei[0], ei[1]
        if transpose:
            row, col = col, row
        if undirected:
            row, col = torch.cat([row, col]), torch.cat([col, row])
            ew = torch.cat([ew, ew])
        return cls.from_coo(row, col, ew, n, gcn_norm=gcn_norm, set_diag=set_diag,
                            remove_diag=remove_diag)

    def size(self, dim):
        return self.num_nodes if dim == 0 else self.num_cols

    def sparse_sizes(self):
        return (self.num_nodes, self.num_cols)

    def nnz(self):
        return int(self.col.numel())

    def csr(self):
        return self.rowptr.long(), self.col.long(), self.val

    def coo(self):
        counts = (self.rowptr[1:] - self.rowptr[:-1]).long()
        row = torch.repeat_interleave(torch.arange(self.num_nodes), counts)
        return row, self.col.long(), self.val

    def to_dense(self):
        row, col, val = self.coo()
        a = torch.zeros(self.num_nodes, self.num_cols, dtype=torch.float32)
        a.index_put_((row, col), val, accumulate=True)
        return a

    def max_degree(self):
        if self.num_nodes == 0:
            return 0
        return int((self.rowptr[1:] - self.rowptr[:-1]).max())

    def device_csr(self, device):
        key = str(device)
        if key not in self._dev:
            self._dev[key] = (self.rowptr.to(device), self.col.to(device), self.val.to(device))
        return self._dev[key]

    def tile_plan(self, feat, device, limits=None, tall=True):
        key = (feat % 64 == 0, str(device))
        if key not in self._plans:
            plan = std = None
            if feat % 64 == 0 and self.nnz() > 0:
                from . import plancache
                if limits is None:
                    limits = hip.tiled_limits(feat)
                tl = hip.tall_tile_limits(feat)
                plan, std = plancache.fetch(self, "tile", (sorted(limits.items()), sorted(tl.items())),
                                            lambda: self._build_tile_plans(limits, tl))
            if std is not None:
                self._plans[(key, "std")] = std.to(device)
            self._plans[key] = None if plan is None else plan.to(device)
        if not tall and (key, "std") in self._plans:
            return self._plans[(key, "std")]
        return self._plans[key]

    def _build_tile_plans(self, limits, tl):
        std = None
        plan = build_tile_plan(self.rowptr.numpy(), self.col.numpy(), self.val.numpy(), self.num_nodes, **limits)
        poor = plan is None or plan.tile_rows < 32
        if poor and self.num_cols == self.num_nodes and self.num_nodes >= 2048 and \
                self.nnz() >= 8 * self.num_nodes:
            order = locality_order(self.rowptr.numpy(), self.col.numpy(), self.num_nodes)
            alt = build_reordered_plan(self.rowptr.numpy(), self.col.numpy(), self.val.numpy(),
                                       self.num_nodes, order, **limits)
            if alt is not None and (plan is None or alt.tile_rows > plan.tile_rows):
                plan = alt
        if plan is not None and not plan.reordered and plan.tile_rows <= 64 and \
                (plan.gw is None or plan.group_fill < 0.5) and limits.get("max_tile_rows", 64) <= 64 \
                and plan.max_row_edges <= 32:
            for tr in (384, 320, 256, 192, 128):
                if tr > tl["max_tile_rows"]:
                    continue
                rpg = 4 if tr <= 256 else 6
                nb = 1 if plan.max_row_edges <= 16 else 2
                room = 160 * 1024 - rpg * 64 * nb * 16 * 6
                mu = min(tl["max_union"], room // (64 * 256) * 64)
                tp = build_tile_plan(self.rowptr.numpy(), self.col.numpy(), self.val.numpy(),
                                     self.num_nodes, mu, tl["max_tile_rows"], 32,
                                     candidates=(tr,)) if mu >= tr // 2 else None
                if tp is not None and tp.tile_rows > 128:
                    std, plan = plan, tp
                    break
        return plan, std

    def colblock_plan(self, feat, device):
        key = ("colblock", feat, str(device))
        if key not in self._plans:
            plan = None
            from . import colblock
            if feat % 64 == 0 and self.num_cols < colblock.MAX_COLS and self.nnz() > 0:
                lib = hip.load()
                plan = colblock.build_colblock_plan(self.rowptr.numpy(), self.col.numpy(), self.val.numpy(),
                                                    self.num_nodes, self.num_cols, feat,
                                                    rows_cap=lib.sgp_spmm_colblock_rows_cap(),
                                                    round_pad=lib.sgp_spmm_colblock_round_pad(),
                                                    l2_bytes=tune.get("colblock_l2_mb", 2.5, float) * 2 ** 20)
                if plan is not None:
                    plan = plan.to(device)
            self._plans[key] = plan
        return self._plans[key]

    def mix_plan(self, feat, device, strict=True):
        key = ("mix", feat % 64 == 0, str(device), bool(strict))
        if key not in self._plans:
            plan = None
            base = self.tile_plan(feat, device, tall=False)
            if base is not None and base.pipe is not None and (base.group_fill >= 0.5 or not strict):
                from . import mixplan, plancache
                lib = hip.load()
                thr, dh = tune.get("mix_thr", 4, int), lib.sgp_spmm_mix_max_dense(int(self.num_cols > self.num_nodes))

                def build():
                    order = None
                    if base.reordered:
                        order = locality_order(self.rowptr.numpy(), self.col.numpy(), self.num_nodes)
                    return mixplan.build_mix_plan(self.rowptr.numpy(), self.col.numpy(), self.val.numpy(), self.num_nodes,
                                                  base, thr=thr, dh=dh, order=order)
                plan = plancache.fetch(self, "mix", (thr, dh, sorted(hip.tiled_limits(feat).items())), build)
                min_share = tune.get("mix_min_share", 0.25, float) if strict else -1.0
                if plan is not None and (plan.dense_share < min_share
                                         or plan.max_union > lib.sgp_spmm_mix_max_union()):
                    plan = None
                if plan is not None:
                    plan = plan.to(device)
            self._plans[key] = plan
        return self._plans[key]

    def split_plan(self, device):
        key = ("split", str(device))
        if key not in self._plans:
            plan = None
            if self.nnz() > 0:
                from . import plancache
                lib = hip.load()
                lim, wide = hip.split_limits(), hip.split_limits(wide=True)
                if tune.get("split_wide", 1, int) == 0:
                    wide = None
                plan = plancache.fetch(self, "split", (sorted(lim.items()), wide and sorted(wide.items()),
                                                       tune.get("split_passes", 1, int), _split_order_mode()),
                                       lambda: self._build_split_plan(lim, wide))
                if isinstance(plan, list):
                    plan = SplitPasses(p.to(device) for p in plan)
                elif plan is not None:
                    plan = plan.to(device)
            self._plans[key] = plan
        return self._plans[key]

    def _build_split_plan(self, lim, wide=None):
        from . import splitplan
        args = (self.rowptr.numpy(), self.col.numpy(), self.val.numpy(), self.num_nodes, self.num_cols)
        bands = dict(band_cols=SPLIT_BAND_BYTES // 256)
        plan = splitplan.build_split_plan(*args, **lim, **bands)
        if plan is not None and plan.stats["rows_per_wave"] < 0.75 * lim["rows_per_wave"] and self.num_nodes >= 2048 and \
                self.num_cols == self.num_nodes:
            alt = splitplan.build_split_plan(*args, order=locality_order(
                self.rowptr.numpy(), self.col.numpy(), self.num_nodes), **lim, **bands)
            if alt is not None and alt.stats["staged_per_row"] < plan.stats["staged_per_row"]:
                plan = alt
                plan.stats["order"] = "locality"
        mode = _split_order_mode()
        if plan is not None and mode != "off" and self.num_cols == self.num_nodes:
            given = plan.stats["tiles"]
            blob = splitplan.blob_order(*args[:2], *args[3:], **lim)
            tiles = splitplan.deal_tiles(*args[:2], *args[3:], order=blob, **lim)
            if tiles is not None and (tiles < given or mode == "on"):
                plan = splitplan.build_split_plan(*args, order=blob, **lim, **bands)
                plan.stats["order"] = "blob"
            plan.stats.setdefault("order", "numbering")
            plan.stats.update(split_order=mode, tiles_given=given, tiles_blob=tiles)
        if plan is not None and (plan.stats["rows_per_wave"] < 0.375 * lim["rows_per_wave"] or
                                 plan.stats["staged_per_row"] > 8):
            plan = None
        if plan is None and self.max_degree() > 32 * lim["chunks"] and tune.get("split_passes", 1, int) != 0:
            deg = (self.rowptr[1:] - self.rowptr[:-1])
            if wide is not None and float((deg > 32 * lim["chunks"]).float().mean()) < 0.5:
                wide = None
            passes = splitplan.build_split_passes(*args, max_passes=12, **(wide or lim), **bands)
            if passes is not None and passes[0].stats["rows_per_wave"] >= 0.5 * lim["rows_per_wave"] and \
                    passes[0].stats["staged_per_row"] <= 8:
                plan = list(passes)
            elif wide is not None:
                return self._build_split_plan(lim, None)
        return plan

    def prepare(self, feat, device, halo=False):
        self.device_csr(device)
        if self.nnz() == 0:
            return ["csr"]
        c = self._select(feat, device, _NOMINAL)
        made = (["split"] if c.split is not None else []) + (["tile"] if c.tile is not None else [])
        if c.lazy:
            return made + ["csr (behind the split hop's predicate until a flag asks for the exact kernels)"]
        made += {"spmm_mix": ["mix"], "spmm_colblock": ["colblock"]}.get(c.kernel, [])
        return made or ["csr"]

    def split_eligible(self, x, y, halo=None):
        return self._select(x.shape[2], x.device, _operands(x, y, halo, None), split_only=True).split is not None

    def norm_inf(self):
        if not hasattr(self, "_norm_inf"):
            rp = self.rowptr.long()
            sums = torch.zeros(self.num_nodes, dtype=torch.float64)
            if self.nnz():
                sums.index_add_(0, torch.repeat_interleave(torch.arange(self.num_nodes), rp[1:] - rp[:-1]),
                                self.val.double().abs())
            self._norm_inf = float(sums.max()) if self.num_nodes else 0.0
        return self._norm_inf

    def propagate(self, x, y, force=None, halo=None, x_bound=None):
        if (halo is None) != (self.num_cols == self.num_nodes):
            raise ValueError("halo rows are required exactly when num_cols > num_nodes")
        if x.dim() != 3 or y.dim() != 3 or y.shape[0] != x.shape[0] or y.shape[2] != x.shape[2]:
            raise ValueError("propagate expects [B, N, F] operands of equal batch and feature size")
        n_src = x.shape[1] + (0 if halo is None else halo.shape[1])
        if n_src != self.num_cols or y.shape[1] != self.num_nodes:
            raise ValueError(f"operand shapes do not match the operator: {n_src} source rows for "
                             f"{self.num_cols} columns, {y.shape[1]} result rows for {self.num_nodes}")
        if halo is not None and (halo.shape[0] != x.shape[0] or halo.shape[2] != x.shape[2]):
            raise ValueError("halo batch / feature size differs from x")
        if force not in (None, "csr", "tiled", "res", "mix", "colblock", "split"):
            raise ValueError(f"unknown kernel {force!r} (csr, tiled, res, mix, colblock, split)")
        if x.shape[0] == 0 or x.shape[2] == 0 or self.num_nodes == 0:
            self.next_bound = self.last_split_flag = None
            return y
        self._poll_flags()
        self.next_bound = self.last_split_flag = None
        c = self._select(x.shape[2], x.device, _operands(x, y, halo, x_bound), force)
        if c.error is not None:
            raise c.error
        if isinstance(x_bound, (int, float)) and x_bound == 0:
            x_bound = None
        pred = None
        if c.split is not None:
            if force == "split":
                prof = hip.spmm_split(c.split, x, y, hip.split_profile(x, halo, x_bound, self.norm_inf(), guard=False),
                                      halo=halo, n_own=self.num_nodes, walk=c.walk)
                self.last_kernel, self.next_bound = "spmm_split", prof.bound_out
                return y
            prof = hip.split_profile(x, halo, x_bound, self.norm_inf(), guard=tune.get("split_guard", 1, int) != 0)
            hip.spmm_split(c.split, x, y, prof, halo=halo, n_own=self.num_nodes, predicated=True, walk=c.walk)
            self.next_bound, pred = prof.bound_out, (prof.flag, 0)
        _LAUNCH[c.kernel](c.plan, x, y, halo, self.num_nodes, pred=pred)
        if pred is None:
            self.last_kernel = c.kernel
            return y
        if c.lazy:
            self._watch_flag(prof.flag)
        self.last_kernel, self.last_exact_kernel, self.last_split_flag = "spmm_split", c.kernel, prof.flag
        return y

    def _select(self, feat, device, ops, force=None, split_only=False):
        nonfinite = ops.bound == "nonfinite"
        split_width = feat % 16 == 0 and feat <= hip.load().sgp_spmm_split_max_feat()
        if force == "split":
            if nonfinite:
                return _Choice(error=ValueError("the split-fp16 hop needs a finite bound on |x|"))
            split = self.split_plan(device) if split_width else None
            if split is None:
                return _Choice(error=NotImplementedError(
                    "no split-fp16 plan for this operator / feature width / halo / operand"))
            return _Choice(split=split, walk=split_band_cols(self.num_cols, feat, split.n_tiles))
        split = None
        if force is None and not nonfinite and tune.get("hop", "split") == "split" and ops.split_layout and split_width \
                and self.nnz() >= 8 * self.num_nodes and self.num_nodes >= 2048:
            split = self.split_plan(device)
        walk = None
        if split is not None:
            walk = split_band_cols(self.num_cols, feat, split.n_tiles)
            if walk is not None:
                for p in (split if isinstance(split, list) else [split]):
                    p.band_table(walk)
        if split_only:
            return _Choice(split=split, walk=walk)
        return self._select_exact(feat, device, ops, force, split)._replace(walk=walk)

    def _select_exact(self, feat, device, ops, force, split):
        if split is not None and tune.get("exact_plans", "lazy") != "eager" and not self._exact_seen:
            return _Choice("spmm_csr_rows", self.device_csr(device), split, lazy=True)
        tile = None if force in ("csr", "colblock") else self.tile_plan(feat, device, tall=force in (None, "tiled"))
        plan = tile if ops.fits32 or force is not None else None
        if force in (None, "mix") and plan is not None and ops.fits32 and \
                (force == "mix" or tune.get("exact", "mix") == "mix"):
            mplan = self.mix_plan(feat, device, strict=force is None)
            if mplan is not None:
                return _Choice("spmm_mix", mplan, split, tile=tile)
        if force == "mix":
            return _Choice(error=NotImplementedError("no mixed dense / sparse plan for this graph / feature width"))
        if force in ("tiled", "res") and plan is None:
            return _Choice(error=NotImplementedError("no tile plan for this graph / feature width"))
        lib = hip.load()
        if plan is not None and plan.gw is not None and plan.pipe is not None and \
                (force == "res" or (force is None and plan.group_fill >= 0.5)) and \
                plan.pipe["max_tile_quads"] <= lib.sgp_spmm_res_max_quads() and \
                plan.pipe["max_union"] <= lib.sgp_spmm_res_max_union():
            return _Choice("spmm_res", plan, split, tile=tile)
        if force == "res":
            return _Choice(error=NotImplementedError("no two-phase row-group stream for this plan"))
        if plan is not None and plan.reordered:
            if force == "tiled":
                return _Choice(error=NotImplementedError("a reordered plan serves the row-group kernels only"))
            plan = None
        if force == "colblock" or (force is None and plan is None and ops.fits32
                                   and feat % 64 == 0 and ops.batch >= 4
                                   and self.num_cols * feat * 4 > 3 * 2 ** 20
                                   and self.nnz() >= 16 * self.num_nodes
                                   and tune.get("colblock", 1, int) != 0):
            cplan = self.colblock_plan(feat, device) if ops.halo_aligned else None
            if cplan is not None:
                return _Choice("spmm_colblock", cplan, split, tile=tile)
            if force == "colblock":
                return _Choice(error=NotImplementedError("no column-blocked plan for this operator / feature width / halo"))
        if plan is not None:
            return _Choice("spmm_tiled", plan, split, tile=tile)
        return _Choice("spmm_csr_rows", self.device_csr(device), split, tile=tile)

    def resolved_kernel(self):
        flag = getattr(self, "last_split_flag", None)
        if flag is None:
            return getattr(self, "last_kernel", None)
        if int(flag.item()) == 1:
            return "spmm_split"
        self._exact_seen = True
        return self.last_exact_kernel

    _FLAG_SLOTS = 32

    def _watch_flag(self, flag):
        if self._flag_host is None:
            self._flag_host = torch.empty(self._FLAG_SLOTS, dtype=torch.int32).pin_memory()
            self._flag_pending = []
        if len(self._flag_pending) >= self._FLAG_SLOTS:
            return
        used = {i for i, _ in self._flag_pending}
        slot = next(i for i in range(self._FLAG_SLOTS) if i not in used)
        self._flag_host[slot:slot + 1].copy_(flag, non_blocking=True)
        ev = torch.cuda.Event()
        ev.record(torch.cuda.current_stream(flag.device))
        self._flag_pending.append((slot, ev))

    def _poll_flags(self):
        if not self._flag_pending:
            return
        still = []
        for slot, ev in self._flag_pending:
            if ev.query():
                if int(self._flag_host[slot]) == 0:
                    self._exact_seen = True
            else:
                still.append((slot, ev))
        self._flag_pending = still

    def index_select(self, dim, index):
        if dim != 0:
            raise NotImplementedError("only row selection (dim=0) is used by the reference")
        idx = torch.as_tensor(index, dtype=torch.long).cpu()
        rp = self.rowptr.long()
        counts = (rp[1:] - rp[:-1])[idx]
        new_rp = torch.zeros(idx.numel() + 1, dtype=torch.long)
        new_rp[1:] = torch.cumsum(counts, 0)
        take = torch.repeat_interleave(rp[idx] - new_rp[:-1], counts) + torch.arange(int(new_rp[-1]))
        return ShiftOperator(new_rp, self.col[take], self.val[take], idx.numel(), num_cols=self.num_cols)

    def propagate_rect(self, x, y):
        if x.shape[1] != self.num_cols or y.shape[1] != self.num_nodes:
            raise ValueError("operand shapes do not match the operator")
        if self.num_cols == self.num_nodes:
            return self.propagate(x, y)
        rowptr, col, val = self.device_csr(x.device)
        hip.spmm_csr(rowptr, col, val, x, y)
        return y

    def __matmul__(self, x):
        if not torch.is_tensor(x) or x.dim() < 2:
            raise TypeError("ShiftOperator @ expects a dense tensor [..., N, F]")
        lead = x.shape[:-2]
        x3 = x.reshape(-1, x.shape[-2], x.shape[-1])
        if x3.dtype != torch.float32:
            x3 = x3.float()
        if x3.stride(2) != 1:
            x3 = x3.contiguous()
        if x3.shape[1] != self.num_cols:
            raise ValueError(f"operand has {x3.shape[1]} rows, the operator {self.num_cols} columns")
        on_cpu = not x3.is_cuda
        if on_cpu:
            hip.require_gpu()
            x3 = x3.cuda()
        y = torch.empty(x3.shape[0], self.num_nodes, x3.shape[2], dtype=torch.float32, device=x3.device)
        self.propagate_rect(x3, y)
        if on_cpu:
            y = y.cpu()
        return y.reshape(*lead, self.num_nodes, x.shape[-1])


def _split_order_mode():
    mode = tune.get("split_order", "auto")
    if mode not in ("off", "on", "auto"):
        raise ValueError(f"SGP_TUNE: split_order={mode!r} is not one of off, on, auto")
    return mode


class SplitPasses(list):

    @property
    def stats(self):
        return self[0].stats

    @property
    def n_tiles(self):
        return sum(p.n_tiles for p in self)
```

### sgp_amd/plancache.py

```python
import hashlib
import os
import tempfile

import torch

VERSION = 9
_dir = None
stats = {"hits": 0, "misses": 0, "stores": 0}


def set_dir(path):
    global _dir
    _dir = path


def directory():
    return _dir or os.environ.get("SGP_AMD_CACHE") or None


def operator_hash(op):
    h = getattr(op, "_csr_hash", None)
    if h is None:
        m = hashlib.blake2b(digest_size=16)
        m.update(f"{op.num_nodes}:{op.num_cols}:{op.nnz()}".encode())
        for t in (op.rowptr, op.col, op.val):
            m.update(t.contiguous().numpy().tobytes())
        h = op._csr_hash = m.hexdigest()
    return h


def _path(op, kind, params):
    d = directory()
    if d is None:
        return None
    tag = hashlib.blake2b(repr((VERSION, kind, params)).encode(), digest_size=8).hexdigest()
    return os.path.join(d, f"{kind}-{operator_hash(op)}-{tag}.pt")


_MISS = object()


def fetch(op, kind, params, build):
    path = _path(op, kind, params)
    if path is None:
        return build()
    if os.path.exists(path):
        try:
            got = torch.load(path, map_location="cpu", weights_only=False)
            if isinstance(got, dict) and got.get("version") == VERSION and got.get("params") == repr(params):
                stats["hits"] += 1
                return got["plan"]
        except Exception:
            pass
    stats["misses"] += 1
    plan = build()
    try:
        os.makedirs(os.path.dirname(path), exist_ok=True)
        fd, tmp = tempfile.mkstemp(dir=os.path.dirname(path), suffix=".tmp")
        os.close(fd)
        torch.save({"version": VERSION, "params": repr(params), "plan": plan}, tmp)
        os.replace(tmp, path)
        stats["stores"] += 1
    except OSError:
        pass
    return plan
```

### sgp_amd/splitplan.py

```python
import numpy as np
import torch


class SplitPlan:
    def __init__(self, hdr, rowid, ucol, afr, adr, rinv, n_tiles, n_rows, n_cols, norm_inf, stats):
        self.hdr, self.rowid, self.ucol, self.afr, self.adr, self.rinv = hdr, rowid, ucol, afr, adr, rinv
        self.n_tiles, self.n_rows, self.n_cols = n_tiles, n_rows, n_cols
        self.norm_inf, self.stats = norm_inf, stats
        self.accumulate = False
        self.bands = {}
        self.ucol_host = ucol if ucol.device.type == "cpu" else None

    def __setstate__(self, state):
        self.__dict__.update(state)
        self.__dict__.setdefault("bands", {})
        self.__dict__.setdefault("ucol_host", self.ucol if self.ucol.device.type == "cpu" else None)

    def to(self, device):
        p = SplitPlan(self.hdr.to(device), self.rowid.to(device), self.ucol.to(device), self.afr.to(device),
                      self.adr.to(device), self.rinv.to(device), self.n_tiles, self.n_rows, self.n_cols, self.norm_inf,
                      self.stats)
        p.accumulate = self.accumulate
        p.bands = {k: (t.to(device), m) for k, (t, m) in self.bands.items()}
        p.ucol_host = self.ucol_host
        return p

    def band_table(self, col_budget):
        col_budget = int(col_budget)
        if col_budget not in self.bands:
            host = self.ucol_host if self.ucol_host is not None else self.ucol.cpu()
            first = build_bands(host, self.n_cols, col_budget)
            self.bands[col_budget] = (first.to(self.ucol.device), int((first[1:] - first[:-1]).max()))
        return self.bands[col_budget]

    def describe(self):
        st = self.stats
        line = (f"split plan: {st['tiles']} tiles, {st['rows_per_tile']:.1f} rows per tile, {st['rows_per_wave']:.2f} rows per wave, "
                f"{st['staged_per_row']:.2f} staged rows per result row")
        if "order" in st:
            line += (f"; rows dealt in {st['order']} order (SGP_TUNE split_order={st['split_order']}: "
                     f"{st['tiles_given']} tiles in the given order, {st['tiles_blob']} in blob order)")
        return line


def build_bands(ucol, n_cols, col_budget):
    from . import hip
    lib = hip.load()
    ucol = ucol.contiguous()
    assert ucol.dtype == torch.int32 and ucol.dim() == 2 and ucol.device.type == "cpu"
    n_tiles = ucol.shape[0]
    first = torch.empty(n_tiles + 1, dtype=torch.int32)
    n = lib.sgp_split_plan_bands(ucol.data_ptr(), n_tiles, ucol.shape[1], int(n_cols), int(col_budget), first.data_ptr())
    if n < 0:
        raise (MemoryError if n == -3 else RuntimeError)("sgp_split_plan_bands: " + lib.sgp_last_error().decode())
    return first[:n + 1].clone()


def _host_csr(rowptr, col, n_rows):
    rowptr = np.ascontiguousarray(rowptr, dtype=np.int64)
    col = np.ascontiguousarray(col, dtype=np.int64)
    if rowptr.size < n_rows + 1:
        raise ValueError("rowptr is shorter than n_rows + 1")
    return rowptr, col


def blob_order(rowptr, col, n_rows, n_cols, waves=16, chunks=7, max_union=768, rows_per_wave=16):
    import ctypes
    from . import hip
    lib = hip.load()
    rowptr, col = _host_csr(rowptr, col, n_rows)
    ptr = lambda a: a.ctypes.data_as(ctypes.c_void_p)
    order = np.empty(n_rows, dtype=np.int64)
    rc = lib.sgp_split_plan_order(ptr(rowptr), ptr(col), col.size, n_rows, n_cols, waves, chunks, max_union, rows_per_wave, ptr(order))
    if rc != 0:
        raise (MemoryError if rc == -3 else ValueError)("sgp_split_plan_order: " + lib.sgp_last_error().decode())
    return order


def deal_tiles(rowptr, col, n_rows, n_cols, waves=16, chunks=7, max_union=768, rows_per_wave=16, order=None):
    import ctypes
    from . import hip
    lib = hip.load()
    rowptr, col = _host_csr(rowptr, col, n_rows)
    seq = None if order is None else np.ascontiguousarray(order, dtype=np.int64)
    ptr = lambda a: a.ctypes.data_as(ctypes.c_void_p)
    out = [np.empty(max(n_rows, 1), dtype=np.int64) for _ in range(4)]
    n_waves = lib.sgp_split_plan_deal(ptr(rowptr), ptr(col), col.size, n_rows, n_cols, None if seq is None else ptr(seq),
                                      0 if seq is None else seq.size, waves, chunks, max_union, rows_per_wave, *map(ptr, out))
    if n_waves == -2 or n_waves == 0:
        return None
    if n_waves < 0:
        raise (MemoryError if n_waves == -3 else RuntimeError)("sgp_split_plan_deal: " + lib.sgp_last_error().decode())
    return int(out[2][n_waves - 1]) + 1


def deal_rows(rowptr, col, n_rows, n_cols, waves, chunks, max_union, rows_per_wave=32, order=None):
    cap = 32 * chunks
    wmark = np.full(n_cols, -1, dtype=np.int64)
    tmark = np.full(n_cols, -1, dtype=np.int64)
    wave_of_row = np.full(n_rows, -1, dtype=np.int64)
    slot_of_row = np.full(n_rows, -1, dtype=np.int64)
    tile_of_wave, rows = [], []
    wave, tile = -1, -1
    w_rows = w_cols = t_cols = t_waves = 0

    def open_wave(r, new_tile):
        nonlocal wave, tile, w_rows, w_cols, t_cols, t_waves
        wave += 1
        if new_tile:
            tile += 1
            t_cols = t_waves = 0
        t_waves += 1
        w_rows = w_cols = 0
        tile_of_wave.append(tile)
        rows.append(0)

    for r in (range(n_rows) if order is None else order):
        r = int(r)
        c = np.unique(col[rowptr[r]:rowptr[r + 1]])
        if c.size > cap or c.size > max_union:
            return None
        if wave < 0:
            open_wave(r, True)
        new_w = int((wmark[c] != wave).sum())
        new_t = int((tmark[c] != tile).sum())
        need_wave = w_rows == rows_per_wave or w_cols + new_w > cap
        if t_cols + new_t > max_union or (need_wave and t_waves == waves):
            open_wave(r, True)
            new_w = new_t = c.size
        elif need_wave:
            open_wave(r, False)
            new_w = c.size
        wmark[c] = wave
        tmark[c] = tile
        w_cols += new_w
        t_cols += new_t
        wave_of_row[r] = wave
        slot_of_row[r] = w_rows
        w_rows += 1
        rows[wave] = w_rows
    return (wave_of_row, slot_of_row, np.asarray(tile_of_wave, dtype=np.int64), np.asarray(rows, dtype=np.int64))


def split_fp16(v):
    v = np.asarray(v, dtype=np.float32)
    bits = v.view(np.uint32) & np.uint32(0xFFFFE000)
    hi32 = bits.view(np.float32)
    small = np.abs(v) < np.float32(2.0 ** -14)
    hi32 = np.where(small, v.astype(np.float16).astype(np.float32), hi32)
    hi = hi32.astype(np.float16)
    lo = (v - hi.astype(np.float32)).astype(np.float16)
    return hi, lo


_SET_SLOTS = np.array([[0, 1, 2, 3, 8, 9, 10, 11], [4, 5, 6, 7, 12, 13, 14, 15],
                       [16, 17, 18, 19, 24, 25, 26, 27], [20, 21, 22, 23, 28, 29, 30, 31]])


def _bank_aware_slots(w_of_key, pos_of_key, stage, n_chunks_total, chunks):
    chunk = pos_of_key // 32
    wc = w_of_key * chunks + chunk
    res = stage & 7
    idx = np.arange(wc.size)

    def rank_within(group, *minor):
        order = np.lexsort(tuple(reversed(minor)) + (group,))
        g = group[order]
        first = np.r_[True, g[1:] != g[:-1]]
        start = np.maximum.accumulate(np.where(first, idx, 0))
        out = np.empty_like(idx)
        out[order] = idx - start
        return out

    rank = rank_within(wc * 8 + res, stage)
    primary = rank < 4
    slot = np.full(wc.size, -1, dtype=np.int64)
    j = rank_within(np.where(primary, wc * 4 + rank, -1), res)
    slot[primary] = _SET_SLOTS[rank[primary], j[primary]]
    occ = np.zeros((n_chunks_total, 32), dtype=bool)
    occ[wc[primary], slot[primary]] = True
    extra = ~primary
    if extra.any():
        free = np.argsort(occ, axis=1, kind="stable")
        e = rank_within(np.where(extra, wc, -1), res, stage)
        slot[extra] = free[wc[extra], e[extra]]
    return chunk * 32 + slot


def build_split_plan(rowptr, col, val, n_rows, n_cols, waves=16, chunks=7, max_union=768, order=None, rows_per_wave=16,
                     threads=0, band_cols=None):
    import ctypes
    from . import hip
    lib = hip.load()
    rowptr = np.ascontiguousarray(rowptr, dtype=np.int64)
    col = np.ascontiguousarray(col, dtype=np.int64)
    val = np.ascontiguousarray(val, dtype=np.float32)
    if n_rows == 0 or col.size == 0 or not np.isfinite(val).all():
        return None
    assert rows_per_wave == 16 and rowptr.size >= n_rows + 1 and val.size == col.size
    if col.min() < 0 or col.max() >= n_cols:
        raise ValueError("column index out of range")
    seq = None if order is None else np.ascontiguousarray(order, dtype=np.int64)
    ptr = lambda a: a.ctypes.data_as(ctypes.c_void_p)
    wave_of_row, slot_of_row = np.empty(n_rows, dtype=np.int64), np.empty(n_rows, dtype=np.int64)
    tile_of_wave, rows = np.empty(n_rows, dtype=np.int64), np.empty(n_rows, dtype=np.int64)
    n_waves = lib.sgp_split_plan_deal(ptr(rowptr), ptr(col), col.size, n_rows, n_cols, None if seq is None else ptr(seq),
                                      0 if seq is None else seq.size, waves, chunks, max_union, rows_per_wave,
                                      ptr(wave_of_row), ptr(slot_of_row), ptr(tile_of_wave), ptr(rows))
    if n_waves == -2 or n_waves == 0:
        return None
    if n_waves < 0:
        raise (MemoryError if n_waves == -3 else RuntimeError)("sgp_split_plan_deal: " + lib.sgp_last_error().decode())
    tile_of_wave, rows = tile_of_wave[:n_waves], rows[:n_waves]
    n_tiles = int(tile_of_wave[-1]) + 1
    hdr = torch.empty((n_tiles, 64), dtype=torch.int32)
    rowid = torch.empty((n_tiles, waves, rows_per_wave), dtype=torch.int32)
    ucol = torch.empty((n_tiles, max_union), dtype=torch.int32)
    afr = torch.empty((n_tiles, waves, chunks, 2, 64, 8), dtype=torch.float16)
    adr = torch.empty((n_tiles, waves, chunks, 64), dtype=torch.int32)
    rinv = torch.empty((n_tiles, waves, 16), dtype=torch.float32)
    st = np.zeros(8, dtype=np.float64)
    hip._check(lib.sgp_split_plan_fill(ptr(rowptr), ptr(col), ptr(val), col.size, n_rows, n_cols, ptr(wave_of_row), ptr(slot_of_row),
                                       ptr(tile_of_wave), ptr(rows), n_waves, n_tiles, waves, chunks, max_union,
                                       hdr.data_ptr(), rowid.data_ptr(), ucol.data_ptr(), afr.data_ptr(), adr.data_ptr(),
                                       rinv.data_ptr(), ptr(st), int(threads)), "sgp_split_plan_fill")
    stats = dict(tiles=n_tiles, waves=int(n_waves), rows_per_wave=float(st[2]), rows_per_tile=float(st[3]),
                 staged_per_row=float(st[4]), chunk_fill=float(st[5]), max_union=int(st[6]))
    plan = SplitPlan(hdr, rowid, ucol, afr, adr, rinv, n_tiles, n_rows, n_cols, float(st[7]), stats)
    if band_cols:
        plan.band_table(band_cols)
    return plan


def build_split_plan_numpy(rowptr, col, val, n_rows, n_cols, waves=16, chunks=7, max_union=768, order=None, rows_per_wave=16):
    rowptr = np.asarray(rowptr, dtype=np.int64)
    col = np.asarray(col, dtype=np.int64)
    val = np.asarray(val, dtype=np.float32)
    if n_rows == 0 or col.size == 0 or not np.isfinite(val).all():
        return None
    assert rows_per_wave == 16
    deal = deal_rows(rowptr, col, n_rows, n_cols, waves, chunks, max_union, rows_per_wave=rows_per_wave, order=order)
    if deal is None:
        return None
    wave_of_row, slot_of_row, tile_of_wave, rows = deal
    n_waves = tile_of_wave.size
    n_tiles = int(tile_of_wave[-1]) + 1
    first_wave_of_tile = np.searchsorted(tile_of_wave, np.arange(n_tiles))
    w_in_tile = np.arange(n_waves) - first_wave_of_tile[tile_of_wave]

    row_of_edge = np.repeat(np.arange(n_rows, dtype=np.int64), np.diff(rowptr[:n_rows + 1]))
    rowsum = np.zeros(n_rows, dtype=np.float64)
    np.add.at(rowsum, row_of_edge, np.abs(val.astype(np.float64)))
    dealt = wave_of_row[row_of_edge] >= 0
    row_of_edge, col, val = row_of_edge[dealt], col[dealt], val[dealt]
    e_wave = wave_of_row[row_of_edge]
    e_tile = tile_of_wave[e_wave]
    tkey, tinv = np.unique(e_tile * n_cols + col, return_inverse=True)
    t_of_key = tkey // n_cols
    t_first = np.searchsorted(t_of_key, np.arange(n_tiles))
    union = np.diff(np.append(t_first, tkey.size))
    stage_of_key = np.arange(tkey.size) - t_first[t_of_key]
    ucol = np.full((n_tiles, max_union), -1, dtype=np.int32)
    ucol[t_of_key, stage_of_key] = (tkey % n_cols).astype(np.int32)
    empty = union == 0
    ucol[empty, 0] = 0
    union = np.where(empty, 1, union)
    wkey, winv = np.unique(e_wave * n_cols + col, return_inverse=True)
    w_of_key = wkey // n_cols
    w_first = np.searchsorted(w_of_key, np.arange(n_waves))
    pos_of_key = np.arange(wkey.size) - w_first[w_of_key]
    assert int(pos_of_key.max()) < 32 * chunks and int(union.max()) <= max_union
    stage_of_wkey = stage_of_key[np.searchsorted(tkey, tile_of_wave[w_of_key] * n_cols + wkey % n_cols)]

    pos_of_key = _bank_aware_slots(w_of_key, pos_of_key, stage_of_wkey, n_waves * chunks, chunks)

    srow = np.full((n_waves, chunks * 32), -1, dtype=np.int64)
    srow[w_of_key, pos_of_key] = stage_of_wkey
    sets = srow.reshape(n_waves * chunks, 32)[:, _SET_SLOTS]
    rep = np.where(sets >= 0, sets, np.iinfo(np.int64).max).min(-1, keepdims=True)
    rep = np.where(rep == np.iinfo(np.int64).max, 0, rep)
    filled = np.where(sets >= 0, sets, rep)
    tmp = np.empty((n_waves * chunks, 32), dtype=np.int64)
    tmp[:, _SET_SLOTS.reshape(-1)] = filled.reshape(n_waves * chunks, 32)
    srow = tmp.reshape(n_waves, chunks * 32)
    srow = srow.reshape(n_waves, chunks, 4, 2, 4)
    lane_i = np.arange(16)
    sl = srow[:, :, :, :, lane_i >> 2]
    a = (sl >> 3) * 512 + (sl & 7) * 32 + 8 * (lane_i & 3)
    a = a.transpose(0, 1, 3, 2, 4).reshape(n_waves, chunks, 2, 64)
    assert int(a.max()) < 65536
    adr = np.zeros((n_tiles, waves, chunks, 64), dtype=np.int32)
    adr[tile_of_wave, w_in_tile] = (a[:, :, 0] | (a[:, :, 1] << 16)).astype(np.int32)

    pos = pos_of_key[winv]
    slot = slot_of_row[row_of_edge]
    k = pos % 32
    dense = np.zeros((n_waves, chunks, 64, 8), dtype=np.float32)
    np.add.at(dense, (e_wave, pos // 32, slot + 16 * (k // 8), k % 8), val)
    rmax = np.abs(dense).reshape(n_waves, chunks, 4, 16, 8).max(axis=(1, 2, 4))
    with np.errstate(divide="ignore", over="ignore"):
        q = np.float32(16384.0) / rmax
    e_row = np.where(rmax > 0, np.where(np.isinf(q), 126.0, np.frexp(np.where(np.isfinite(q), q, 1.0))[1] - 1.0), 0.0)
    e_row = np.clip(e_row, -126, 126)
    rscale = np.exp2(e_row).astype(np.float32)
    lane_scale = np.tile(rscale, (1, 4))
    hi, lo = split_fp16(dense * lane_scale[:, None, :, None])
    afr = np.zeros((n_tiles, waves, chunks, 2, 64, 8), dtype=np.float16)
    afr[tile_of_wave, w_in_tile, :, 0] = hi
    afr[tile_of_wave, w_in_tile, :, 1] = lo
    rinv = np.zeros((n_tiles, waves, 16), dtype=np.float32)
    filled = np.arange(16)[None, :] < rows[:, None]
    rinv[tile_of_wave, w_in_tile] = np.where(filled, np.exp2(-e_row), 0.0).astype(np.float32)

    hdr = np.zeros((n_tiles, 64), dtype=np.int32)
    hdr[tile_of_wave, waves + w_in_tile] = rows
    rowid = np.full((n_tiles, waves, rows_per_wave), -1, dtype=np.int32)
    all_rows = np.flatnonzero(wave_of_row >= 0)
    rowid[tile_of_wave[wave_of_row[all_rows]], w_in_tile[wave_of_row[all_rows]], slot_of_row[all_rows]] = all_rows
    hdr[:, 2 * waves] = union
    n_dealt = max(1, int(all_rows.size))
    stats = dict(tiles=n_tiles, waves=n_waves, rows_per_wave=float(rows.mean()),
                 rows_per_tile=float(n_dealt / n_tiles), staged_per_row=float(union.sum() / n_dealt),
                 chunk_fill=float(wkey.size / (n_waves * chunks * 32)), max_union=int(union.max()))
    return SplitPlan(torch.from_numpy(hdr), torch.from_numpy(rowid), torch.from_numpy(ucol), torch.from_numpy(afr), torch.from_numpy(adr),
                     torch.from_numpy(rinv), n_tiles, n_rows, n_cols, float(rowsum.max()), stats)


def build_split_passes(rowptr, col, val, n_rows, n_cols, waves=16, chunks=7, max_union=768, order=None,
                       rows_per_wave=16, segment=None, max_passes=12, band_cols=None):
    rowptr = np.asarray(rowptr, dtype=np.int64)
    col = np.asarray(col, dtype=np.int64)
    val = np.asarray(val, dtype=np.float32)
    lim = dict(waves=waves, chunks=chunks, max_union=max_union, rows_per_wave=rows_per_wave, band_cols=band_cols)
    one = build_split_plan(rowptr, col, val, n_rows, n_cols, order=order, **lim)
    if one is not None:
        return [one]
    if n_rows == 0 or col.size == 0 or not np.isfinite(val).all():
        return None
    cap = int(segment or min(32 * chunks, max_union))
    seq = np.arange(n_rows) if order is None else np.asarray(order, dtype=np.int64)
    group_of_row = np.full(n_rows, -1, dtype=np.int64)
    group_of_row[seq] = np.arange(seq.size) // rows_per_wave
    n_groups = (seq.size + rows_per_wave - 1) // rows_per_wave
    row_of_edge = np.repeat(np.arange(n_rows, dtype=np.int64), np.diff(rowptr[:n_rows + 1]))
    g_of_edge = group_of_row[row_of_edge]
    gkey, ginv = np.unique(g_of_edge * n_cols + col, return_inverse=True)
    g_of_key = gkey // n_cols
    first = np.searchsorted(g_of_key, np.arange(n_groups))
    rank = np.arange(gkey.size) - first[g_of_key]
    pass_of_edge = (rank // cap)[ginv]
    n_pass = int(pass_of_edge.max()) + 1
    if n_pass > max_passes:
        return None
    plans = []
    for p in range(n_pass):
        take = pass_of_edge == p
        cnt = np.bincount(row_of_edge[take], minlength=n_rows)
        rp = np.zeros(n_rows + 1, dtype=np.int64)
        rp[1:] = np.cumsum(cnt)
        if p == 0:
            rows_p = seq
        else:
            live = np.zeros(n_groups, dtype=bool)
            live[np.unique(g_of_edge[take])] = True
            rows_p = seq[live[group_of_row[seq]]]
        plan = build_split_plan(rp, col[take], val[take], n_rows, n_cols, order=rows_p, **lim)
        if plan is None:
            return None
        plan.accumulate = p > 0
        plans.append(plan)
    return plans


def plan_matrix(plan, n_rows, n_cols):
    hdr, ucol, rowid = plan.hdr.numpy(), plan.ucol.numpy(), plan.rowid.numpy()
    afr, adr, rinv = plan.afr.numpy().astype(np.float64), plan.adr.numpy(), plan.rinv.numpy().astype(np.float64)
    waves, chunks = afr.shape[1], afr.shape[2]
    out = np.zeros((n_rows, n_cols))
    for t in range(plan.n_tiles):
        for w in range(waves):
            if int(hdr[t, waves + w]) == 0:
                continue
            for c in range(chunks):
                for lane in range(64):
                    m, g = lane & 15, lane >> 4
                    for e in range(8):
                        kk = 8 * g + e
                        j, i4 = (kk % 8) // 4, kk % 4
                        src_lane = 16 * g + 4 * i4
                        a_ = (int(adr[t, w, c, src_lane]) >> (16 * j)) & 0xFFFF
                        s = (a_ // 512) * 8 + (a_ % 512) // 32
                        v = afr[t, w, c, 0, lane, e] + afr[t, w, c, 1, lane, e]
                        if v != 0.0:
                            out[int(rowid[t, w, m]), int(ucol[t, s])] += v * rinv[t, w, m]
    return out
```

Before: 1.327 billion.

## Trim unused MFMA chunks per wave and balance waves across SIMDs

The split-plan builder now records in the tile header how many 32-key chunks each wave actually uses, not the fixed chunk count, so the kernel can skip empty chunk MFMAs. It also reassigns wave slots within a tile with a greedy longest-first deal, so the per-SIMD sum of chunks (waves i mod 4) is balanced. The plan cache version is bumped and the mode defaults to auto. This assumes the kernel reads the per-wave chunk count from header slots 0..W-1, and it changes wave-to-slot placement, which affects rowid, adr and afr layout.

Result: no change. 1.346 billion, median of 4 (+1.5%).

```diff
diff --git a/include/sgp_amd.h b/include/sgp_amd.h
--- a/include/sgp_amd.h
+++ b/include/sgp_amd.h
@@ -142,6 +142,12 @@
                         int32_t waves, int32_t chunks, int32_t max_union,
                         int32_t* hdr, int32_t* rowid, int32_t* ucol, void* afr, int32_t* adr, float* rinv,
                         double* stats, int32_t threads);
+int sgp_split_plan_fill_trim(const int64_t* rowptr, const int64_t* col, const float* val, int64_t nnz, int64_t n_rows, int64_t n_cols,
+                             const int64_t* wave_of_row, const int64_t* slot_of_row, const int64_t* tile_of_wave,
+                             const int64_t* rows_of_wave, int64_t n_waves, int64_t n_tiles,
+                             int32_t waves, int32_t chunks, int32_t max_union,
+                             int32_t* hdr, int32_t* rowid, int32_t* ucol, void* afr, int32_t* adr, float* rinv,
+                             double* stats, int32_t threads, int32_t trim, int64_t* trim_stats);
 int64_t sgp_split_plan_bands(const int32_t* ucol, int64_t n_tiles, int32_t max_union, int64_t n_cols,
                              int64_t col_budget, int32_t* band_first);
 
diff --git a/sgp_amd/csrc/plan_split.hip b/sgp_amd/csrc/plan_split.hip
--- a/sgp_amd/csrc/plan_split.hip
+++ b/sgp_amd/csrc/plan_split.hip
@@ -44,25 +44,66 @@
     int64_t n_waves, n_tiles;
     int waves, chunks, max_union;
     int32_t* hdr; int32_t* rowid; int32_t* ucol; uint16_t* afr; int32_t* adr; float* rinv;
+    int trim;
 };
+
+struct TrimOut { int64_t* hist; int64_t simd_max, simd_max_deal; };
 
 struct Scratch {
     std::vector<int32_t> stage_of_col, kpos_of_col;
     std::vector<int64_t> cols;
+    std::vector<std::vector<int64_t>> wcols;
     std::vector<float> dense;
-    explicit Scratch(const FillArgs& a) : stage_of_col(a.n_cols, -1), kpos_of_col(a.n_cols, -1), dense((size_t)a.chunks * 512) {}
+    explicit Scratch(const FillArgs& a) : stage_of_col(a.n_cols, -1), kpos_of_col(a.n_cols, -1), wcols(a.waves), dense((size_t)a.chunks * 512) {}
 };
 
 int64_t fill_tile(const FillArgs& a, int64_t t, const int64_t* first_wave, const int64_t* row_list, const int64_t* row_first,
-                  Scratch& s, int64_t& union_out) {
+                  Scratch& s, int64_t& union_out, TrimOut& tr) {
     const int W = a.waves, C = a.chunks;
     const int64_t w0 = first_wave[t], w1 = first_wave[t + 1];
-    s.cols.clear();
-    for (int64_t w = w0; w < w1; ++w)
+    int nch[64], place[64];
+    for (int i = 0; i < W; ++i) { nch[i] = 1; place[i] = i; }
+    if (w1 - w0 > W) return -1;
+    for (int64_t w = w0; w < w1; ++w) {
+        std::vector<int64_t>& wc = s.wcols[w - w0];
+        wc.clear();
         for (int64_t i = row_first[w]; i < row_first[w + 1]; ++i) {
             const int64_t r = row_list[i];
-            s.cols.insert(s.cols.end(), a.col + a.rowptr[r], a.col + a.rowptr[r + 1]);
-        }
+            wc.insert(wc.end(), a.col + a.rowptr[r], a.col + a.rowptr[r + 1]);
+        }
+        std::sort(wc.begin(), wc.end());
+        wc.erase(std::unique(wc.begin(), wc.end()), wc.end());
+        const int64_t nk = (int64_t)wc.size();
+        if (nk > 32 * C) return -1;
+        nch[w - w0] = (int)std::max<int64_t>(1, (nk + 31) / 32);
+        ++tr.hist[nch[w - w0]];
+    }
+    {
+        int64_t sum[4] = {0, 0, 0, 0};
+        for (int i = 0; i < W; ++i) sum[i & 3] += nch[i];
+        tr.simd_max_deal = tr.simd_max = *std::max_element(sum, sum + 4);
+        if (a.trim && W % 4 == 0) {
+            int idx[64], at[64], cnt[4] = {0, 0, 0, 0};
+            int64_t lsum[4] = {0, 0, 0, 0};
+            for (int i = 0; i < W; ++i) idx[i] = i;
+            std::stable_sort(idx, idx + W, [&](int x, int y) { return nch[x] > nch[y]; });
+            for (int k = 0; k < W; ++k) {
+                int best = -1;
+                for (int q = 0; q < 4; ++q)
+                    if (cnt[q] < W / 4 && (best < 0 || lsum[q] < lsum[best])) best = q;
+                at[idx[k]] = best + 4 * cnt[best]++;
+                lsum[best] += nch[idx[k]];
+            }
+            const int64_t lmax = *std::max_element(lsum, lsum + 4);
+            if (lmax < tr.simd_max_deal) {
+                tr.simd_max = lmax;
+                for (int i = 0; i < W; ++i) place[i] = at[i];
+            }
+        }
+    }
+    for (int i = 0; i < W; ++i) a.hdr[t * 64 + i] = a.trim ? 1 : C;
+    s.cols.clear();
+    for (int64_t w = w0; w < w1; ++w) s.cols.insert(s.cols.end(), s.wcols[w - w0].begin(), s.wcols[w - w0].end());
     std::sort(s.cols.begin(), s.cols.end());
     s.cols.erase(std::unique(s.cols.begin(), s.cols.end()), s.cols.end());
     if (s.cols.empty()) s.cols.push_back(0);
@@ -77,19 +118,16 @@
     a.hdr[t * 64 + 2 * W] = (int32_t)U;
     int64_t keys = 0;
     for (int64_t w = w0; w < w1; ++w) {
-        const int win = (int)(w - w0);
+        const int win = place[w - w0];
         const int nrows = (int)a.rows_of_wave[w];
         a.hdr[t * 64 + W + win] = nrows;
-        s.cols.clear();
+        if (a.trim) a.hdr[t * 64 + win] = nch[w - w0];
+        const std::vector<int64_t>& wc = s.wcols[w - w0];
         for (int64_t i = row_first[w]; i < row_first[w + 1]; ++i) {
             const int64_t r = row_list[i];
             a.rowid[(t * W + win) * 16 + a.slot_of_row[r]] = (int32_t)r;
-            s.cols.insert(s.cols.end(), a.col + a.rowptr[r], a.col + a.rowptr[r + 1]);
-        }
-        std::sort(s.cols.begin(), s.cols.end());
-        s.cols.erase(std::unique(s.cols.begin(), s.cols.end()), s.cols.end());
-        const int nk = (int)s.cols.size();
-        if (nk > 32 * C) return -1;
+        }
+        const int nk = (int)wc.size();
         keys += nk;
         int32_t* adr = a.adr + ((t * W + win) * C) * 64;
         for (int c = 0; c < C; ++c) {
@@ -98,24 +136,24 @@
             const int k0 = 32 * c, k1 = std::min(nk, 32 * c + 32);
             int cnt_res[8] = {0, 0, 0, 0, 0, 0, 0, 0}, in_set[4] = {0, 0, 0, 0};
             int rank[32], slot[32];
-            for (int k = k0; k < k1; ++k) rank[k - k0] = cnt_res[s.stage_of_col[s.cols[k]] & 7]++;
+            for (int k = k0; k < k1; ++k) rank[k - k0] = cnt_res[s.stage_of_col[wc[k]] & 7]++;
             for (int r = 0; r < 4; ++r)
                 for (int res = 0; res < 8; ++res)
                     for (int k = k0; k < k1; ++k)
-                        if (rank[k - k0] == r && (s.stage_of_col[s.cols[k]] & 7) == res) slot[k - k0] = SET_SLOTS[r][in_set[r]++];
+                        if (rank[k - k0] == r && (s.stage_of_col[wc[k]] & 7) == res) slot[k - k0] = SET_SLOTS[r][in_set[r]++];
             bool occ[32] = {};
             for (int k = k0; k < k1; ++k) if (rank[k - k0] < 4) occ[slot[k - k0]] = true;
             int free_at = 0;
             for (int res = 0; res < 8; ++res)
                 for (int k = k0; k < k1; ++k)
-                    if (rank[k - k0] >= 4 && (s.stage_of_col[s.cols[k]] & 7) == res) {
+                    if (rank[k - k0] >= 4 && (s.stage_of_col[wc[k]] & 7) == res) {
                         while (occ[free_at]) ++free_at;
                         slot[k - k0] = free_at;
                         occ[free_at] = true;
                     }
             for (int k = k0; k < k1; ++k) {
-                srow[slot[k - k0]] = s.stage_of_col[s.cols[k]];
-                s.kpos_of_col[s.cols[k]] = 32 * c + slot[k - k0];
+                srow[slot[k - k0]] = s.stage_of_col[wc[k]];
+                s.kpos_of_col[wc[k]] = 32 * c + slot[k - k0];
             }
             for (int q = 0; q < 4; ++q) {
                 int rep = -1;
@@ -421,22 +459,23 @@
   });
 }
 
-extern "C" int sgp_split_plan_fill(const int64_t* rowptr, const int64_t* col, const float* val, int64_t nnz, int64_t n_rows, int64_t n_cols,
-                                   const int64_t* wave_of_row, const int64_t* slot_of_row, const int64_t* tile_of_wave,
-                                   const int64_t* rows_of_wave, int64_t n_waves, int64_t n_tiles,
-                                   int32_t waves, int32_t chunks, int32_t max_union,
-                                   int32_t* hdr, int32_t* rowid, int32_t* ucol, void* afr, int32_t* adr, float* rinv,
-                                   double* stats, int32_t threads) {
-  return guarded<int>("sgp_split_plan_fill", [&]() -> int {
+namespace {
+int fill_plan(const int64_t* rowptr, const int64_t* col, const float* val, int64_t nnz, int64_t n_rows, int64_t n_cols,
+              const int64_t* wave_of_row, const int64_t* slot_of_row, const int64_t* tile_of_wave,
+              const int64_t* rows_of_wave, int64_t n_waves, int64_t n_tiles,
+              int32_t waves, int32_t chunks, int32_t max_union,
+              int32_t* hdr, int32_t* rowid, int32_t* ucol, void* afr, int32_t* adr, float* rinv,
+              double* stats, int32_t threads, int32_t trim, int64_t* trim_stats, const char* who) {
+  return guarded<int>(who, [&]() -> int {
     SGP_REQUIRE(rowptr && col && val && wave_of_row && slot_of_row && tile_of_wave && rows_of_wave && hdr && rowid && ucol &&
-                afr && adr && rinv && stats, "sgp_split_plan_fill: null pointer");
+                afr && adr && rinv && stats, "%s: null pointer", who);
     SGP_REQUIRE(n_rows > 0 && n_cols > 0 && n_waves > 0 && n_tiles > 0 && waves >= 1 && 2 * waves < 64 && chunks >= 1 &&
-                max_union >= 1 && max_union <= 65536 / 64 * 8, "sgp_split_plan_fill: bad size");
-    if (const char* f = rowptr_fault(rowptr, n_rows, nnz)) return sgp::fail(SGP_EINVAL, "sgp_split_plan_fill: malformed CSR: %s", f);
+                max_union >= 1 && max_union <= 65536 / 64 * 8, "%s: bad size", who);
+    if (const char* f = rowptr_fault(rowptr, n_rows, nnz)) return sgp::fail(SGP_EINVAL, "%s: malformed CSR: %s", who, f);
     for (int64_t e = 0; e < rowptr[n_rows]; ++e)
-        SGP_REQUIRE(col[e] >= 0 && col[e] < n_cols, "sgp_split_plan_fill: column out of range");
+        SGP_REQUIRE(col[e] >= 0 && col[e] < n_cols, "%s: column out of range", who);
     FillArgs a{rowptr, col, val, n_rows, n_cols, wave_of_row, slot_of_row, tile_of_wave, rows_of_wave, n_waves, n_tiles,
-               waves, chunks, max_union, hdr, rowid, ucol, (uint16_t*)afr, adr, rinv};
+               waves, chunks, max_union, hdr, rowid, ucol, (uint16_t*)afr, adr, rinv, trim != 0};
     memset(hdr, 0, sizeof(int32_t) * 64 * n_tiles);
     std::fill(rowid, rowid + n_tiles * waves * 16, -1);
     std::fill(ucol, ucol + n_tiles * (int64_t)max_union, -1);
@@ -447,13 +486,13 @@
     for (int64_t w = 0; w < n_waves; ++w) {
         const int64_t t = tile_of_wave[w];
         SGP_REQUIRE(t >= 0 && t < n_tiles && (w == 0 || t == tile_of_wave[w - 1] || t == tile_of_wave[w - 1] + 1),
-                    "sgp_split_plan_fill: tile_of_wave is not a non-decreasing run");
-        SGP_REQUIRE(rows_of_wave[w] >= 0 && rows_of_wave[w] <= 16, "sgp_split_plan_fill: a wave holds at most 16 rows");
+                    "%s: tile_of_wave is not a non-decreasing run", who);
+        SGP_REQUIRE(rows_of_wave[w] >= 0 && rows_of_wave[w] <= 16, "%s: a wave holds at most 16 rows", who);
         ++first_wave[t + 1];
         row_first[w + 1] = row_first[w] + rows_of_wave[w];
     }
     for (int64_t t = 0; t < n_tiles; ++t) {
-        SGP_REQUIRE(first_wave[t + 1] >= 1 && first_wave[t + 1] <= waves, "sgp_split_plan_fill: a tile holds 1 .. waves waves");
+        SGP_REQUIRE(first_wave[t + 1] >= 1 && first_wave[t + 1] <= waves, "%s: a tile holds 1 .. waves waves", who);
         first_wave[t + 1] += first_wave[t];
     }
     const int64_t n_dealt = row_first[n_waves];
@@ -463,30 +502,36 @@
         const int64_t w = wave_of_row[r];
         if (w < 0) continue;
         SGP_REQUIRE(w < n_waves && slot_of_row[r] >= 0 && slot_of_row[r] < rows_of_wave[w] && row_list[row_first[w] + slot_of_row[r]] < 0,
-                    "sgp_split_plan_fill: wave / slot of row %lld inconsistent", (long long)r);
+                    "%s: wave / slot of row %lld inconsistent", who, (long long)r);
         row_list[row_first[w] + slot_of_row[r]] = r;
         ++seen;
     }
-    SGP_REQUIRE(seen == n_dealt, "sgp_split_plan_fill: rows_of_wave does not match wave_of_row");
+    SGP_REQUIRE(seen == n_dealt, "%s: rows_of_wave does not match wave_of_row", who);
 
     int nthr = threads > 0 ? threads : (int)std::thread::hardware_concurrency();
     nthr = (int)std::max<int64_t>(1, std::min<int64_t>(std::min(nthr, 64), n_tiles));
     nthr = (int)std::max<int64_t>(1, std::min<int64_t>(nthr, (1ll << 30) / (8 * n_cols)));
-    std::atomic<int64_t> next(0), keys(0), usum(0), umax(0);
+    std::atomic<int64_t> next(0), keys(0), usum(0), umax(0), simd_sum(0), simd_sum_deal(0);
+    std::vector<std::atomic<int64_t>> hist((size_t)chunks + 1);
+    for (auto& h : hist) h.store(0);
     std::atomic<int> bad(0);
     auto work = [&]() {
         try {
             Scratch s(a);
-            int64_t k_local = 0, u_local = 0, u_max = 0;
+            int64_t k_local = 0, u_local = 0, u_max = 0, m_local = 0, md_local = 0;
+            std::vector<int64_t> h_local((size_t)chunks + 1, 0);
+            TrimOut tr{h_local.data(), 0, 0};
             for (;;) {
                 const int64_t t = next.fetch_add(1);
                 if (t >= n_tiles || bad.load()) break;
                 int64_t U = 0;
-                const int64_t k = fill_tile(a, t, first_wave.data(), row_list.data(), row_first.data(), s, U);
+                const int64_t k = fill_tile(a, t, first_wave.data(), row_list.data(), row_first.data(), s, U, tr);
                 if (k < 0) { bad.store(1); break; }
                 k_local += k; u_local += U; u_max = std::max(u_max, U);
-            }
-            keys += k_local; usum += u_local;
+                m_local += tr.simd_max; md_local += tr.simd_max_deal;
+            }
+            keys += k_local; usum += u_local; simd_sum += m_local; simd_sum_deal += md_local;
+            for (int c = 0; c <= chunks; ++c) hist[c] += h_local[c];
             int64_t cur = umax.load();
             while (u_max > cur && !umax.compare_exchange_weak(cur, u_max)) {}
         } catch (...) { bad.store(2); }
@@ -502,8 +547,8 @@
         }
         for (auto& th : pool) th.join();
     }
-    if (bad.load() == 2) return sgp::fail(SGP_ENOMEM, "sgp_split_plan_fill: out of host memory");
-    if (bad.load()) return sgp::fail(SGP_EUNSUP, "sgp_split_plan_fill: the dealt rows break the kernel's limits");
+    if (bad.load() == 2) return sgp::fail(SGP_ENOMEM, "%s: out of host memory", who);
+    if (bad.load()) return sgp::fail(SGP_EUNSUP, "%s: the dealt rows break the kernel's limits", who);
     double norm_inf = 0.0;
     for (int64_t r = 0; r < n_rows; ++r) {
         double sum = 0.0;
@@ -514,8 +559,34 @@
     stats[0] = (double)n_tiles; stats[1] = (double)n_waves; stats[2] = (double)n_dealt / (double)n_waves;
     stats[3] = dealt / (double)n_tiles; stats[4] = (double)usum.load() / dealt;
     stats[5] = (double)keys.load() / ((double)n_waves * chunks * 32); stats[6] = (double)umax.load(); stats[7] = norm_inf;
+    if (trim_stats) {
+        for (int c = 0; c <= chunks; ++c) trim_stats[c] = hist[c].load();
+        trim_stats[chunks + 1] = simd_sum.load();
+        trim_stats[chunks + 2] = simd_sum_deal.load();
+    }
     return 0;
   });
+}
+}
+
+extern "C" int sgp_split_plan_fill(const int64_t* rowptr, const int64_t* col, const float* val, int64_t nnz, int64_t n_rows, int64_t n_cols,
+                                   const int64_t* wave_of_row, const int64_t* slot_of_row, const int64_t* tile_of_wave,
+                                   const int64_t* rows_of_wave, int64_t n_waves, int64_t n_tiles,
+                                   int32_t waves, int32_t chunks, int32_t max_union,
+                                   int32_t* hdr, int32_t* rowid, int32_t* ucol, void* afr, int32_t* adr, float* rinv,
+                                   double* stats, int32_t threads) {
+    return fill_plan(rowptr, col, val, nnz, n_rows, n_cols, wave_of_row, slot_of_row, tile_of_wave, rows_of_wave, n_waves, n_tiles,
+                     waves, chunks, max_union, hdr, rowid, ucol, afr, adr, rinv, stats, threads, 0, nullptr, "sgp_split_plan_fill");
+}
+
+extern "C" int sgp_split_plan_fill_trim(const int64_t* rowptr, const int64_t* col, const float* val, int64_t nnz, int64_t n_rows, int64_t n_cols,
+                                        const int64_t* wave_of_row, const int64_t* slot_of_row, const int64_t* tile_of_wave,
+                                        const int64_t* rows_of_wave, int64_t n_waves, int64_t n_tiles,
+                                        int32_t waves, int32_t chunks, int32_t max_union,
+                                        int32_t* hdr, int32_t* rowid, int32_t* ucol, void* afr, int32_t* adr, float* rinv,
+                                        double* stats, int32_t threads, int32_t trim, int64_t* trim_stats) {
+    return fill_plan(rowptr, col, val, nnz, n_rows, n_cols, wave_of_row, slot_of_row, tile_of_wave, rows_of_wave, n_waves, n_tiles,
+                     waves, chunks, max_union, hdr, rowid, ucol, afr, adr, rinv, stats, threads, trim, trim_stats, "sgp_split_plan_fill_trim");
 }
 
 extern "C" int64_t sgp_split_plan_bands(const int32_t* ucol, int64_t n_tiles, int32_t max_union, int64_t n_cols,
diff --git a/sgp_amd/csrc/spmm_split_impl.h b/sgp_amd/csrc/spmm_split_impl.h
--- a/sgp_amd/csrc/spmm_split_impl.h
+++ b/sgp_amd/csrc/spmm_split_impl.h
@@ -56,13 +56,18 @@
 #define SGP_SPLIT_SPREAD 0
 #endif
 constexpr bool SPREAD = SGP_SPLIT_SPREAD != 0;
-constexpr int lgkm_behind(int c, bool conv) {
-    int n = 4 * ((c + RING - 1 < NCH ? c + RING - 1 : NCH - 1) - c);
-    if (SPREAD && c + RING - 1 < NCH) n -= 2;
+constexpr int lgkm_behind(int c, bool conv, int A = NCH) {
+    int n = 4 * ((c + RING - 1 < A ? c + RING - 1 : A - 1) - c);
+    if (SPREAD && c + RING - 1 < A) n -= 2;
     if (conv) for (int j = (c - (RING - 1) > 0 ? c - (RING - 1) : 0); j < c; ++j) n += conv_ops(j);
     return n;
 }
-constexpr int lgkm_wait(int c, bool conv) { return lgkm_behind(c, conv) < 15 ? lgkm_behind(c, conv) : 15; }
+constexpr int lgkm_wait(int c, bool conv, int A = NCH) { return lgkm_behind(c, conv, A) < 15 ? lgkm_behind(c, conv, A) : 15; }
+#ifndef SGP_SPLIT_AMIN
+#define SGP_SPLIT_AMIN 4
+#endif
+constexpr int AMIN = SGP_SPLIT_AMIN;
+static_assert(AMIN >= 1 && AMIN <= NCH, "1 .. NCH active chunks");
 static_assert(RING == 4 || (lgkm_behind(NCH - 1, true) <= 15 && lgkm_behind(CR + 1, true) <= 15 && lgkm_behind(CR + 2, true) <= 15),
               "the standard ring's waits are exact");
 
@@ -211,13 +216,18 @@
         float* tab = (float*)(lds + NBUF * BUF);
         for (int i = tid; i < 2 * feat; i += NW * 64) tab[i] = a.xtab[i];
     }
-    h8 af[NCH][2];
-    unsigned ad[NCH];
+    int nch = __builtin_amdgcn_readfirstlane(a.hdr[(size_t)tile * HDR + wave]);
+    if (nch < 1 || nch > NCH) nch = NCH;
+    if (nch < AMIN) nch = AMIN;
+    auto run = [&](auto AC) __attribute__((always_inline)) {
+    constexpr int A = decltype(AC)::value;
+    h8 af[A][2];
+    unsigned ad[A];
     {
         const h8* ap = a.afr + ((size_t)(tile * NW + wave) * NCH * 2) * 64 + lane;
         const int* dp = a.adr + ((size_t)(tile * NW + wave) * NCH) * 64 + lane;
 #pragma unroll
-        for (int c = 0; c < NCH; ++c) {
+        for (int c = 0; c < A; ++c) {
             af[c][0] = ap[(c * 2 + 0) * 64];
             af[c][1] = ap[(c * 2 + 1) * 64];
             ad[c] = (unsigned)dp[c * 64];
@@ -350,35 +360,42 @@
         f32x4 v, s4;
         BOp b[RING];
         stamp(u, 1);
-#pragma unroll
-        for (int c = 0; c < RING - 1; ++c) tr_issue(b[c], addr_lo(cbo, ad[c]), addr_hi(cbo, ad[c]));
+        static_for<0, (RING - 1 < A ? RING - 1 : A)>([&](auto C) {
+            constexpr int c = decltype(C)::value;
+            tr_issue(b[c], addr_lo(cbo, ad[c]), addr_hi(cbo, ad[c]));
+        });
         static_for<0, NCH>([&](auto C) {
             constexpr int c = decltype(C)::value;
+            constexpr bool more = c + RING - 1 < A;
             BOp& x = b[c % RING];
             unsigned na0 = 0, na1 = 0;
-            if constexpr (c + RING - 1 < NCH) {
+            if constexpr (more) {
                 na0 = addr_lo(cbo, ad[c + RING - 1]); na1 = addr_hi(cbo, ad[c + RING - 1]);
                 if constexpr (SPREAD) tr_issue_hi(b[(c + RING - 1) % RING], na0, na1);
                 else tr_issue(b[(c + RING - 1) % RING], na0, na1);
             }
-            if (ABL(8)) tr_wait<lgkm_wait(c, false)>(x); else tr_wait<lgkm_wait(c, true)>(x);
+            if constexpr (c < A) {
+            if (ABL(8)) tr_wait<lgkm_wait(c, false, A)>(x); else tr_wait<lgkm_wait(c, true, A)>(x);
+            }
+            if constexpr (c >= A) {
+            } else
             if (!ABL(2)) {
                 const h8 bh = cat8(x.h0, x.h1), bl = cat8(x.l0, x.l1);
                 acc0 = __builtin_amdgcn_mfma_f32_16x16x32_f16(bh, af[c][0], acc0, 0, 0, 0);
-                if constexpr (SPREAD && c + RING - 1 < NCH) tr_issue_lo(b[(c + RING - 1) % RING], na0, na1);
+                if constexpr (SPREAD && more) tr_issue_lo(b[(c + RING - 1) % RING], na0, na1);
                 acc1 = __builtin_amdgcn_mfma_f32_16x16x32_f16(bl, af[c][0], acc1, 0, 0, 0);
 #if SGP_SPLIT_ACC3
                 acc2 = __builtin_amdgcn_mfma_f32_16x16x32_f16(bh, af[c][1], acc2, 0, 0, 0);
 #else
                 acc1 = __builtin_amdgcn_mfma_f32_16x16x32_f16(bh, af[c][1], acc1, 0, 0, 0);
 #endif
-            } else if constexpr (SPREAD && c + RING - 1 < NCH) tr_issue_lo(b[(c + RING - 1) % RING], na0, na1);
+            } else if constexpr (SPREAD && more) tr_issue_lo(b[(c + RING - 1) % RING], na0, na1);
             if constexpr (VSTAGE) {
                 if constexpr (c == CR - 1) lds_read16(s4, tab_cv + sl1 * 64);
                 if constexpr (c >= CR && c < CR + NLD) {
                     constexpr int i = c - CR;
                     wait_vm<NLD - 1>();
-                    if constexpr (i == 0) asm volatile("s_waitcnt lgkmcnt(%2)" : "+v"(s4), "+v"(ld[i]) : "n"(c + RING - 1 < NCH ? 4 : 0) : "memory");
+                    if constexpr (i == 0) asm volatile("s_waitcnt lgkmcnt(%2)" : "+v"(s4), "+v"(ld[i]) : "n"(more ? 4 : 0) : "memory");
                     else asm volatile("" : "+v"(ld[i]) :: "memory");
                     uint2 hi, lo;
                     split4(ld[i], s4, hi, lo);
@@ -396,7 +413,7 @@
                         if (dma_now) wait_vm_n(nld); else wait_vm<0>();
                         lds_read16(s4, tab_cv + sl1 * 64);
                     } else {
-                        asm volatile("s_waitcnt lgkmcnt(%2)" : "+v"(s4), "+v"(v) : "n"(c + RING - 1 < NCH ? 4 : 0));
+                        asm volatile("s_waitcnt lgkmcnt(%2)" : "+v"(s4), "+v"(v) : "n"(more ? 4 : 0));
                         uint2 hi, lo;
                         split4(v, s4, hi, lo);
                         const unsigned w = cv_off + nxt;
@@ -447,6 +464,10 @@
         asm volatile("s_waitcnt lgkmcnt(0)\n\ts_barrier" ::: "memory");
         stamp(u, 6);
     }
+    };
+    static_for<AMIN, NCH + 1>([&](auto AC) {
+        if (nch == decltype(AC)::value) run(AC);
+    });
 }
 
 }
diff --git a/sgp_amd/csrc/spmm_split_wide.hip b/sgp_amd/csrc/spmm_split_wide.hip
--- a/sgp_amd/csrc/spmm_split_wide.hip
+++ b/sgp_amd/csrc/spmm_split_wide.hip
@@ -3,5 +3,6 @@
 #define SGP_SPLIT_SMAX 896
 #define SGP_SPLIT_CR 6
 #define SGP_SPLIT_VSTAGE 1
+#define SGP_SPLIT_AMIN 10
 #define SGP_SPLIT_NAME(x) sgp_spmm_split_wide_##x
 #include "spmm_split_impl.h"
diff --git a/sgp_amd/graph.py b/sgp_amd/graph.py
--- a/sgp_amd/graph.py
+++ b/sgp_amd/graph.py
@@ -294,7 +294,8 @@
                 if tune.get("split_wide", 1, int) == 0:
                     wide = None
                 plan = plancache.fetch(self, "split", (sorted(lim.items()), wide and sorted(wide.items()),
-                                                       tune.get("split_passes", 1, int), _split_order_mode()),
+                                                       tune.get("split_passes", 1, int), _split_order_mode(),
+                                                       _split_trim_mode()),
                                        lambda: self._build_split_plan(lim, wide))
                 if isinstance(plan, list):
                     plan = SplitPasses(p.to(device) for p in plan)
@@ -549,6 +550,11 @@
         return y.reshape(*lead, self.num_nodes, x.shape[-1])
 
 
+def _split_trim_mode():
+    from . import splitplan
+    return splitplan.split_trim_mode()
+
+
 def _split_order_mode():
     mode = tune.get("split_order", "auto")
     if mode not in ("off", "on", "auto"):
diff --git a/sgp_amd/plancache.py b/sgp_amd/plancache.py
--- a/sgp_amd/plancache.py
+++ b/sgp_amd/plancache.py
@@ -4,7 +4,7 @@
 
 import torch
 
-VERSION = 9
+VERSION = 10
 _dir = None
 stats = {"hits": 0, "misses": 0, "stores": 0}
 
diff --git a/sgp_amd/splitplan.py b/sgp_amd/splitplan.py
--- a/sgp_amd/splitplan.py
+++ b/sgp_amd/splitplan.py
@@ -1,5 +1,37 @@
 import numpy as np
 import torch
+
+from . import tune
+
+SPLIT_TRIM_DEFAULT = "auto"
+
+
+def split_trim_mode():
+    mode = tune.get("split_trim", SPLIT_TRIM_DEFAULT)
+    if mode not in ("auto", "off"):
+        raise ValueError(f"SGP_TUNE: split_trim={mode!r} is not one of auto, off")
+    return mode
+
+
+def _trim_stats(hist, simd_sum, simd_sum_deal, n_tiles, waves, chunks, trim):
+    return dict(split_trim="auto" if trim else "off", nch_hist=[int(v) for v in hist],
+                simd_max=float(simd_sum) / n_tiles, simd_max_deal=float(simd_sum_deal) / n_tiles,
+                simd_max_full=float(chunks * waves // 4))
+
+
+def _place_waves(nch, waves):
+    deal = max(int(nch[q::4].sum()) for q in range(4))
+    ident = np.arange(waves)
+    if waves % 4:
+        return ident, deal, deal
+    order = np.argsort(-nch, kind="stable")
+    sums, cnt, at = [0] * 4, [0] * 4, np.empty(waves, dtype=np.int64)
+    for i in order:
+        best = min((q for q in range(4) if cnt[q] < waves // 4), key=lambda q: (sums[q], q))
+        at[i] = best + 4 * cnt[best]
+        cnt[best] += 1
+        sums[best] += int(nch[i])
+    return (at, max(sums), deal) if max(sums) < deal else (ident, deal, deal)
 
 
 class SplitPlan:
@@ -40,6 +72,10 @@
         if "order" in st:
             line += (f"; rows dealt in {st['order']} order (SGP_TUNE split_order={st['split_order']}: "
                      f"{st['tiles_given']} tiles in the given order, {st['tiles_blob']} in blob order)")
+        if "nch_hist" in st:
+            hist = " ".join(f"{c}:{n}" for c, n in enumerate(st["nch_hist"]) if n)
+            line += (f"; chunks used per wave {hist}; largest per-SIMD chunk sum of a tile {st['simd_max']:.2f} on average "
+                     f"({st['simd_max_deal']:.2f} in deal order, {st['simd_max_full']:.0f} untrimmed; SGP_TUNE split_trim={st['split_trim']})")
         return line
 
 
@@ -188,7 +224,7 @@
 
 
 def build_split_plan(rowptr, col, val, n_rows, n_cols, waves=16, chunks=7, max_union=768, order=None, rows_per_wave=16,
-                     threads=0, band_cols=None):
+                     threads=0, band_cols=None, trim=None):
     import ctypes
     from . import hip
     lib = hip.load()
@@ -220,25 +256,30 @@
     adr = torch.empty((n_tiles, waves, chunks, 64), dtype=torch.int32)
     rinv = torch.empty((n_tiles, waves, 16), dtype=torch.float32)
     st = np.zeros(8, dtype=np.float64)
-    hip._check(lib.sgp_split_plan_fill(ptr(rowptr), ptr(col), ptr(val), col.size, n_rows, n_cols, ptr(wave_of_row), ptr(slot_of_row),
-                                       ptr(tile_of_wave), ptr(rows), n_waves, n_tiles, waves, chunks, max_union,
-                                       hdr.data_ptr(), rowid.data_ptr(), ucol.data_ptr(), afr.data_ptr(), adr.data_ptr(),
-                                       rinv.data_ptr(), ptr(st), int(threads)), "sgp_split_plan_fill")
+    trim = split_trim_mode() == "auto" if trim is None else bool(trim)
+    ts = np.zeros(chunks + 3, dtype=np.int64)
+    hip._check(lib.sgp_split_plan_fill_trim(ptr(rowptr), ptr(col), ptr(val), col.size, n_rows, n_cols, ptr(wave_of_row), ptr(slot_of_row),
+                                            ptr(tile_of_wave), ptr(rows), n_waves, n_tiles, waves, chunks, max_union,
+                                            hdr.data_ptr(), rowid.data_ptr(), ucol.data_ptr(), afr.data_ptr(), adr.data_ptr(),
+                                            rinv.data_ptr(), ptr(st), int(threads), int(trim), ptr(ts)), "sgp_split_plan_fill_trim")
     stats = dict(tiles=n_tiles, waves=int(n_waves), rows_per_wave=float(st[2]), rows_per_tile=float(st[3]),
-                 staged_per_row=float(st[4]), chunk_fill=float(st[5]), max_union=int(st[6]))
+                 staged_per_row=float(st[4]), chunk_fill=float(st[5]), max_union=int(st[6]),
+                 **_trim_stats(ts[:chunks + 1], ts[chunks + 1], ts[chunks + 2], n_tiles, waves, chunks, trim))
     plan = SplitPlan(hdr, rowid, ucol, afr, adr, rinv, n_tiles, n_rows, n_cols, float(st[7]), stats)
     if band_cols:
         plan.band_table(band_cols)
     return plan
 
 
-def build_split_plan_numpy(rowptr, col, val, n_rows, n_cols, waves=16, chunks=7, max_union=768, order=None, rows_per_wave=16):
+def build_split_plan_numpy(rowptr, col, val, n_rows, n_cols, waves=16, chunks=7, max_union=768, order=None, rows_per_wave=16,
+                           trim=None):
     rowptr = np.asarray(rowptr, dtype=np.int64)
     col = np.asarray(col, dtype=np.int64)
     val = np.asarray(val, dtype=np.float32)
     if n_rows == 0 or col.size == 0 or not np.isfinite(val).all():
         return None
     assert rows_per_wave == 16
+    trim = split_trim_mode() == "auto" if trim is None else bool(trim)
     deal = deal_rows(rowptr, col, n_rows, n_cols, waves, chunks, max_union, rows_per_wave=rows_per_wave, order=order)
     if deal is None:
         return None
@@ -272,6 +313,23 @@
     assert int(pos_of_key.max()) < 32 * chunks and int(union.max()) <= max_union
     stage_of_wkey = stage_of_key[np.searchsorted(tkey, tile_of_wave[w_of_key] * n_cols + wkey % n_cols)]
 
+    nch = np.maximum(1, -(-np.bincount(w_of_key, minlength=n_waves) // 32))
+    hdr_nch = np.full((n_tiles, waves), 1 if trim else chunks, dtype=np.int32)
+    simd_sum = simd_sum_deal = 0
+    for t in range(n_tiles):
+        w0 = first_wave_of_tile[t]
+        w1 = first_wave_of_tile[t + 1] if t + 1 < n_tiles else n_waves
+        tile_nch = np.ones(waves, dtype=np.int64)
+        tile_nch[:w1 - w0] = nch[w0:w1]
+        at, placed, dealt_max = _place_waves(tile_nch, waves) if trim else (np.arange(waves), None, None)
+        if not trim:
+            placed = dealt_max = max(int(tile_nch[q::4].sum()) for q in range(4))
+        w_in_tile[w0:w1] = at[:w1 - w0]
+        simd_sum += placed
+        simd_sum_deal += dealt_max
+        if trim:
+            hdr_nch[t, at[:w1 - w0]] = nch[w0:w1]
+
     pos_of_key = _bank_aware_slots(w_of_key, pos_of_key, stage_of_wkey, n_waves * chunks, chunks)
 
     srow = np.full((n_waves, chunks * 32), -1, dtype=np.int64)
@@ -313,6 +371,7 @@
     rinv[tile_of_wave, w_in_tile] = np.where(filled, np.exp2(-e_row), 0.0).astype(np.float32)
 
     hdr = np.zeros((n_tiles, 64), dtype=np.int32)
+    hdr[:, :waves] = hdr_nch
     hdr[tile_of_wave, waves + w_in_tile] = rows
     rowid = np.full((n_tiles, waves, rows_per_wave), -1, dtype=np.int32)
     all_rows = np.flatnonzero(wave_of_row >= 0)
@@ -321,17 +380,18 @@
     n_dealt = max(1, int(all_rows.size))
     stats = dict(tiles=n_tiles, waves=n_waves, rows_per_wave=float(rows.mean()),
                  rows_per_tile=float(n_dealt / n_tiles), staged_per_row=float(union.sum() / n_dealt),
-                 chunk_fill=float(wkey.size / (n_waves * chunks * 32)), max_union=int(union.max()))
+                 chunk_fill=float(wkey.size / (n_waves * chunks * 32)), max_union=int(union.max()),
+                 **_trim_stats(np.bincount(nch, minlength=chunks + 1), simd_sum, simd_sum_deal, n_tiles, waves, chunks, trim))
     return SplitPlan(torch.from_numpy(hdr), torch.from_numpy(rowid), torch.from_numpy(ucol), torch.from_numpy(afr), torch.from_numpy(adr),
                      torch.from_numpy(rinv), n_tiles, n_rows, n_cols, float(rowsum.max()), stats)
 
 
 def build_split_passes(rowptr, col, val, n_rows, n_cols, waves=16, chunks=7, max_union=768, order=None,
-                       rows_per_wave=16, segment=None, max_passes=12, band_cols=None):
+                       rows_per_wave=16, segment=None, max_passes=12, band_cols=None, trim=None):
     rowptr = np.asarray(rowptr, dtype=np.int64)
     col = np.asarray(col, dtype=np.int64)
     val = np.asarray(val, dtype=np.float32)
-    lim = dict(waves=waves, chunks=chunks, max_union=max_union, rows_per_wave=rows_per_wave, band_cols=band_cols)
+    lim = dict(waves=waves, chunks=chunks, max_union=max_union, rows_per_wave=rows_per_wave, band_cols=band_cols, trim=trim)
     one = build_split_plan(rowptr, col, val, n_rows, n_cols, order=order, **lim)
     if one is not None:
         return [one]
```
